# ZPP-Robotics/OSQP-Solver

Hardware: AMD Instinct MI355X
Metric: QPs/sec on a 1024-QP batch of box-QPs (n=512, m=1024), OSQP defaults; ADMM iters/sec alongside (higher is better)
Workload: dtype f64

## Files before the change

### include/mi_osqp.h

```cpp
#ifndef MI_OSQP_H
#define MI_OSQP_H

#include <stdint.h>

#ifdef __cplusplus
extern "C" {
#endif

typedef enum {
  MI_OSQP_OK = 0,
  MI_OSQP_ERR_INVALID_DATA = 1,
  MI_OSQP_ERR_INVALID_SETTINGS = 2,
  MI_OSQP_ERR_PATTERN_CHANGED = 3,
  MI_OSQP_ERR_NONCONVEX = 4,
  MI_OSQP_ERR_DEVICE = 5,
  MI_OSQP_ERR_NULL = 6,
  MI_OSQP_ERR_ALLOC = 7
} mi_osqp_error;

typedef enum {
  MI_OSQP_EXIT_OPTIMAL = 0,
  MI_OSQP_EXIT_PRIMAL_INFEASIBLE = 1,
  MI_OSQP_EXIT_DUAL_INFEASIBLE = 2,
  MI_OSQP_EXIT_OPTIMAL_INACCURATE = 3,
// ... 9 lines not shown
typedef struct {
  double  rho;
  double  sigma;
  int64_t scaling;
  int64_t adaptive_rho;
  int64_t adaptive_rho_interval;
  double  adaptive_rho_tolerance;
  int64_t max_iter;
  double  eps_abs;
  double  eps_rel;
  double  eps_prim_inf;
  double  eps_dual_inf;
  double  alpha;
  int64_t scaled_termination;
  int64_t check_termination;
  int64_t warm_start;
  int64_t verbose;
  int64_t polish;
  int64_t polish_refine_iter;
  double  delta;
} mi_osqp_settings;

typedef struct {
  int64_t iter;
  int64_t status_val;
  int64_t exit_code;
  double  obj_val;
  double  pri_res;
  double  dua_res;
  int64_t rho_updates;
  double  rho_estimate;
  double  rho;
  int64_t status_polish;
} mi_osqp_info;

typedef struct {
  int64_t n, m, N, batch, tile, n_tiles;
  int64_t nnz_P_triu, nnz_A, nnz_KKT, nnz_L;
  int64_t n_supernodes, n_blocks;
  int64_t fwd_levels, bwd_levels, fwd_slots, bwd_slots, chk_slots;
  int64_t lds_bytes, threads_per_block;
  int64_t dense_tail_rows, dense_tail_slots;
  double  setup_seconds_host, setup_seconds_factor, setup_seconds_upload;
  int64_t nnz_L_before_tail;
  int64_t solve_groups, solve_group_threads;
  int64_t resident_state, lds_bytes_iterate;
  int64_t pipelined_refactors;
  int64_t resident_factor_steps, lds_bytes_factor;
  int64_t dense_tail_tasks, dense_tail_waves_used, dense_tail_wave_tasks_max;
  int64_t refactor_lanes;
  int64_t iterate_launches_deep_ring, iterate_launches_long_head;
  int64_t runahead_regions, runahead_tiles, runahead_left, runahead_missed;
  int64_t region_priority, region_lane_checks, region_chunks;
} mi_osqp_stats;

typedef struct mi_osqp_solver mi_osqp_solver;
typedef struct mi_osqp_batch  mi_osqp_batch;

void        mi_osqp_default_settings(mi_osqp_settings *s);
const char *mi_osqp_exit_code_name(int64_t exit_code);
const char *mi_osqp_error_name(int64_t err);
const char *mi_osqp_version(void);
const char *mi_osqp_last_error(void);

int mi_osqp_setup(mi_osqp_solver **out, int64_t n, int64_t m,
                  const int64_t *P_colptr, const int64_t *P_rowidx, const double *P_val,
                  const double *q,
                  const int64_t *A_colptr, const int64_t *A_rowidx, const double *A_val,
                  const double *l, const double *u, const mi_osqp_settings *settings);
int mi_osqp_update_A(mi_osqp_solver *h, const int64_t *A_colptr, const int64_t *A_rowidx,
                     const double *A_val);
int mi_osqp_update_bounds(mi_osqp_solver *h, const double *l, const double *u);
int mi_osqp_update_A_bounds(mi_osqp_solver *h, const int64_t *A_colptr, const int64_t *A_rowidx, const double *A_val,
                            const double *l, const double *u);
int mi_osqp_warm_start_x(mi_osqp_solver *h, const double *x);
int mi_osqp_update_q(mi_osqp_solver *h, const double *q);
int mi_osqp_update_P(mi_osqp_solver *h, const int64_t *P_colptr, const int64_t *P_rowidx, const double *P_val);
int mi_osqp_update_P_A(mi_osqp_solver *h, const int64_t *P_colptr, const int64_t *P_rowidx, const double *P_val,
                       const int64_t *A_colptr, const int64_t *A_rowidx, const double *A_val);
int mi_osqp_warm_start_y(mi_osqp_solver *h, const double *y);
int mi_osqp_solve(mi_osqp_solver *h, mi_osqp_info *info);
int mi_osqp_get_primal(mi_osqp_solver *h, double *x_out);
int mi_osqp_get_dual(mi_osqp_solver *h, double *y_out);
int mi_osqp_get_prim_inf_cert(mi_osqp_solver *h, double *dy_out );
int mi_osqp_get_dual_inf_cert(mi_osqp_solver *h, double *dx_out );
int mi_osqp_adjoint(mi_osqp_solver *h, const double *dx, const double *dy, double *dq, double *dP, double *dA, double *dl, double *du,
                    int32_t *status);
int mi_osqp_get_stats(mi_osqp_solver *h, mi_osqp_stats *st);
int mi_osqp_get_settings(mi_osqp_solver *h, mi_osqp_settings *out);
int mi_osqp_update_settings(mi_osqp_solver *h, const mi_osqp_settings *s);
void mi_osqp_free(mi_osqp_solver *h);

int mi_osqp_batch_setup(mi_osqp_batch **out, int64_t B, int64_t n, int64_t m,
                        const int64_t *P_colptr, const int64_t *P_rowidx, const double *P_val,
                        const double *q,
                        const int64_t *A_colptr, const int64_t *A_rowidx, const double *A_val,
                        const double *l, const double *u, const mi_osqp_settings *settings,
                        int64_t device);
int mi_osqp_batch_update_A(mi_osqp_batch *h, const int64_t *A_colptr, const int64_t *A_rowidx,
                           const double *A_val);
int mi_osqp_batch_update_bounds(mi_osqp_batch *h, const double *l, const double *u);
int mi_osqp_batch_update_A_bounds(mi_osqp_batch *h, const int64_t *A_colptr, const int64_t *A_rowidx, const double *A_val,
                                  const double *l, const double *u);
int mi_osqp_batch_warm_start_x(mi_osqp_batch *h, const double *x);
int mi_osqp_batch_update_q(mi_osqp_batch *h, const double *q);
int mi_osqp_batch_update_P(mi_osqp_batch *h, const int64_t *P_colptr, const int64_t *P_rowidx, const double *P_val);
// ... 117 lines not shown
int mi_osqp_multi_batch_update_rho_each(mi_osqp_multi *h, const double *rho );
int mi_osqp_multi_batch_solve(mi_osqp_multi *h);
int mi_osqp_multi_batch_solve_async(mi_osqp_multi *h);
int mi_osqp_multi_batch_wait(mi_osqp_multi *h);
int mi_osqp_multi_batch_get_primal(mi_osqp_multi *h, double *x_out );
int mi_osqp_multi_batch_get_dual(mi_osqp_multi *h, double *y_out );
int mi_osqp_multi_batch_get_info(mi_osqp_multi *h, mi_osqp_info *info );
int mi_osqp_multi_batch_get_prim_inf_cert(mi_osqp_multi *h, double *dy_out );
int mi_osqp_multi_batch_get_dual_inf_cert(mi_osqp_multi *h, double *dx_out );
int64_t mi_osqp_multi_batch_shards(mi_osqp_multi *h);
int mi_osqp_multi_batch_shard(mi_osqp_multi *h, int64_t k, int64_t *device, int64_t *begin, int64_t *end, mi_osqp_batch **handle);
void mi_osqp_multi_batch_free(mi_osqp_multi *h);

int mi_osqp_batch_spmv(mi_osqp_batch *h, const double *d_x, const double *d_y,
                       double *d_Px, double *d_Aty, double *d_Ax, void *stream);
int mi_osqp_batch_kkt_solve(mi_osqp_batch *h, const double *d_rhs, double *d_sol, void *stream);
int mi_osqp_batch_refactor_device(mi_osqp_batch *h);
int mi_osqp_batch_kernel_time(mi_osqp_batch *h, double *avg_ms, int64_t *launches);
int mi_osqp_batch_refactor_time(mi_osqp_batch *h, double *factor_ms, double *tail_ms, int64_t *launches, int64_t *qps);
int mi_osqp_batch_refactor_peak(mi_osqp_batch *h, int64_t *qps, double *factor_ms, double *tail_ms);

int mi_osqp_batch_get_scaling(mi_osqp_batch *h, double *D , double *E , double *c );

int mi_osqp_debug_host_kkt_solve(int64_t n, int64_t m,
                                 const int64_t *P_colptr, const int64_t *P_rowidx, const double *P_val,
                                 const int64_t *A_colptr, const int64_t *A_rowidx, const double *A_val,
                                 const double *l, const double *u, const mi_osqp_settings *settings,
                                 int64_t tile, const double *rhs ,
                                 double *sol_schedule , double *sol_direct ,
                                 mi_osqp_stats *st);

int mi_osqp_debug_host_block_factor(int64_t n, int64_t m,
                                    const int64_t *P_colptr, const int64_t *P_rowidx, const double *P_val,
                                    const int64_t *A_colptr, const int64_t *A_rowidx, const double *A_val,
                                    const double *l, const double *u, const mi_osqp_settings *settings,
                                    double *max_rel_diff_L, double *max_rel_diff_Dinv, int64_t *counts);

int mi_osqp_debug_refactor_chunks(int64_t n_flagged, const int64_t *flagged, int64_t n_active, const int64_t *active, int64_t tile,
                                  int64_t chunk_qps, int64_t max_chunks, int64_t *n_chunks, int64_t *work_begin, int64_t *tiles,
                                  int64_t *tile_begin);

int mi_osqp_debug_region_chunks(int64_t nq, int64_t gw, int64_t n_cus, int64_t *chunk_qps, int64_t *n_chunks);

int mi_osqp_debug_refactor_lanes(int64_t n_flagged, const int64_t *flagged, int64_t n_active, const int64_t *active, int64_t tile,
                                 int64_t chunk_qps, int64_t max_chunks, int64_t kbt, int64_t lanes, int64_t chunk0_first,
                                 int64_t scratch_slots, int64_t *n_lanes, int64_t *lane_of, int64_t *order, int64_t *order_begin,
                                 int64_t *scratch_begin, int64_t *n_waits, int64_t *wait_chunk, int64_t *wait_for);

int mi_osqp_debug_runahead_group(int64_t n_active, const int64_t *tiles, const double *pri_res, const double *dua_res, int64_t size,
                                 int64_t min_active, int64_t *n_group, int64_t *group);

int mi_osqp_debug_iterate_form(int64_t tiles, int64_t has_head, int64_t forced_form, int64_t long_min, int64_t *form);

int mi_osqp_debug_trace_kkt_solve(mi_osqp_batch *h, int32_t which, const double *d_rhs, double *d_sol,
                                  uint32_t *out, int64_t out_capacity_words, int64_t *dims);

#ifdef __cplusplus
}
#endif
#endif
```

### osqp-solver_amd/__init__.py

```python
import ctypes as C
import os

import numpy as np

try:
    import torch
except ImportError:
    torch = None

from . import build as _build

_HERE = os.path.dirname(os.path.abspath(__file__))
_LIB = None

EXIT_NAMES = ["kOptimal", "kPrimalInfeasible", "kDualInfeasible", "kOptimalInaccurate",
              "kPrimalInfeasibleInaccurate", "kDualInfeasibleInaccurate", "kMaxIterations",
              "kInterrupted", "kTimeLimitReached", "kNonConvex", "kUnknown"]
K_OPTIMAL = 0


class Settings(C.Structure):
    _fields_ = [("rho", C.c_double), ("sigma", C.c_double), ("scaling", C.c_int64),
                ("adaptive_rho", C.c_int64), ("adaptive_rho_interval", C.c_int64),
                ("adaptive_rho_tolerance", C.c_double), ("max_iter", C.c_int64),
                ("eps_abs", C.c_double), ("eps_rel", C.c_double), ("eps_prim_inf", C.c_double),
                ("eps_dual_inf", C.c_double), ("alpha", C.c_double), ("scaled_termination", C.c_int64),
                ("check_termination", C.c_int64), ("warm_start", C.c_int64), ("verbose", C.c_int64),
                ("polish", C.c_int64), ("polish_refine_iter", C.c_int64), ("delta", C.c_double)]


class Info(C.Structure):
    _fields_ = [("iter", C.c_int64), ("status_val", C.c_int64), ("exit_code", C.c_int64),
                ("obj_val", C.c_double), ("pri_res", C.c_double), ("dua_res", C.c_double),
                ("rho_updates", C.c_int64), ("rho_estimate", C.c_double), ("rho", C.c_double),
                ("status_polish", C.c_int64)]

    def as_dict(self):
        return {k: getattr(self, k) for k, _ in self._fields_}


class Stats(C.Structure):
    _fields_ = [(k, C.c_int64) for k in
                ("n", "m", "N", "batch", "tile", "n_tiles", "nnz_P_triu", "nnz_A", "nnz_KKT", "nnz_L",
                 "n_supernodes", "n_blocks", "fwd_levels", "bwd_levels", "fwd_slots", "bwd_slots",
                 "chk_slots", "lds_bytes", "threads_per_block", "dense_tail_rows", "dense_tail_slots")] + \
               [(k, C.c_double) for k in ("setup_seconds_host", "setup_seconds_factor", "setup_seconds_upload")] + \
               [("nnz_L_before_tail", C.c_int64), ("solve_groups", C.c_int64), ("solve_group_threads", C.c_int64),
                ("resident_state", C.c_int64), ("lds_bytes_iterate", C.c_int64), ("pipelined_refactors", C.c_int64),
                ("resident_factor_steps", C.c_int64), ("lds_bytes_factor", C.c_int64),
                ("dense_tail_tasks", C.c_int64), ("dense_tail_waves_used", C.c_int64), ("dense_tail_wave_tasks_max", C.c_int64),
                ("refactor_lanes", C.c_int64),
                ("iterate_launches_deep_ring", C.c_int64), ("iterate_launches_long_head", C.c_int64),
                ("runahead_regions", C.c_int64), ("runahead_tiles", C.c_int64), ("runahead_left", C.c_int64),
                ("runahead_missed", C.c_int64),
                ("region_priority", C.c_int64), ("region_lane_checks", C.c_int64), ("region_chunks", C.c_int64)]

    def as_dict(self):
        return {k: getattr(self, k) for k, _ in self._fields_}


class MiOsqpError(RuntimeError):
    def __init__(self, code, where):
        self.code = int(code)
        L = lib()
        msg = L.mi_osqp_error_name(int(code)).decode()
        extra = L.mi_osqp_last_error().decode()
        super().__init__(f"{where}: error {int(code)} ({msg}) {extra}")


def lib():
    global _LIB
    if _LIB is None:
        path = os.path.join(_HERE, "libmi_osqp.so")
        if os.environ.get("MI_OSQP_LIBRARY"):
            path = os.environ["MI_OSQP_LIBRARY"]
        else:
            try:
                path = _build.build()
            except Exception as e:
                if not os.path.exists(path):
                    raise ImportError(f"libmi_osqp.so missing and could not be built: {e}") from e
        L = C.CDLL(path)
        ip, dp, vp = C.POINTER(C.c_int64), C.POINTER(C.c_double), C.c_void_p
        L.mi_osqp_default_settings.argtypes = [C.POINTER(Settings)]
        for f in ("mi_osqp_exit_code_name", "mi_osqp_error_name"):
            getattr(L, f).restype = C.c_char_p; getattr(L, f).argtypes = [C.c_int64]
        L.mi_osqp_version.restype = C.c_char_p
        L.mi_osqp_last_error.restype = C.c_char_p
        L.mi_osqp_batch_setup.argtypes = [C.POINTER(vp), C.c_int64, C.c_int64, C.c_int64, ip, ip, dp, dp, ip, ip, dp,
                                          dp, dp, C.POINTER(Settings), C.c_int64]
        L.mi_osqp_batch_update_A.argtypes = [vp, ip, ip, dp]
        L.mi_osqp_batch_update_A_bounds.argtypes = [vp, ip, ip, dp, dp, dp]
        L.mi_osqp_batch_update_bounds.argtypes = [vp, dp, dp]
        L.mi_osqp_batch_warm_start_x.argtypes = [vp, dp]
        L.mi_osqp_batch_update_q.argtypes = [vp, dp]
        L.mi_osqp_batch_update_q_device.argtypes = [vp, vp, vp]
        L.mi_osqp_batch_update_P.argtypes = [vp, ip, ip, dp]
        L.mi_osqp_batch_update_P_A.argtypes = [vp, ip, ip, dp, ip, ip, dp]
        L.mi_osqp_batch_warm_start_y.argtypes = [vp, dp]
        L.mi_osqp_batch_get_P_upper_pattern.argtypes = [vp, ip, ip, ip]
        L.mi_osqp_batch_update_P_device.argtypes = [vp, vp, vp]
        L.mi_osqp_batch_update_P_A_bounds_device.argtypes = [vp, vp, vp, vp, vp, vp]
        L.mi_osqp_batch_update_P_some.argtypes = [vp, C.c_int64, ip, dp]
        L.mi_osqp_batch_update_P_A_bounds_some.argtypes = [vp, C.c_int64, ip, dp, dp, dp, dp]
        L.mi_osqp_batch_update_q_some.argtypes = [vp, C.c_int64, ip, dp]
        L.mi_osqp_batch_warm_start_y_some.argtypes = [vp, C.c_int64, ip, dp]
        L.mi_osqp_settings_update_check.argtypes = [C.POINTER(Settings), C.POINTER(Settings)]
        L.mi_osqp_batch_get_settings.argtypes = [vp, C.POINTER(Settings)]
# ... 36 lines not shown
        L.mi_osqp_batch_refactor_peak.argtypes = [vp, ip, dp, dp]
        L.mi_osqp_batch_reinit_some.argtypes = [vp, C.c_int64, ip, dp, dp, dp]
        L.mi_osqp_batch_update_A_bounds_some.argtypes = [vp, C.c_int64, ip, dp, dp, dp]
        L.mi_osqp_batch_warm_start_x_some.argtypes = [vp, C.c_int64, ip, dp]
        L.mi_osqp_batch_solve_begin_some.argtypes = [vp, C.c_int64, ip]
        L.mi_osqp_batch_polish_some.argtypes = [vp, C.c_int64, ip]
        L.mi_osqp_batch_advance.argtypes = [vp, C.c_int64]
        L.mi_osqp_batch_poll.argtypes = [vp, C.c_int64, ip, ip, C.c_int64]
        L.mi_osqp_batch_get_primal_some.argtypes = [vp, C.c_int64, ip, dp]
        L.mi_osqp_batch_get_dual_some.argtypes = [vp, C.c_int64, ip, dp]
        L.mi_osqp_batch_get_info_some.argtypes = [vp, C.c_int64, ip, C.POINTER(Info)]
        L.mi_osqp_batch_running.argtypes = [vp]; L.mi_osqp_batch_running.restype = C.c_int64
        L.mi_osqp_batch_ring_wraps.argtypes = [vp]; L.mi_osqp_batch_ring_wraps.restype = C.c_int64
        L.mi_osqp_release_device_cache.argtypes = []; L.mi_osqp_release_device_cache.restype = None
        L.mi_osqp_setup.argtypes = [C.POINTER(vp), C.c_int64, C.c_int64, ip, ip, dp, dp, ip, ip, dp, dp, dp, C.POINTER(Settings)]
        L.mi_osqp_update_A.argtypes = [vp, ip, ip, dp]
        L.mi_osqp_update_bounds.argtypes = [vp, dp, dp]
        L.mi_osqp_warm_start_x.argtypes = [vp, dp]
        L.mi_osqp_update_q.argtypes = [vp, dp]
        L.mi_osqp_update_P.argtypes = [vp, ip, ip, dp]
        L.mi_osqp_update_P_A.argtypes = [vp, ip, ip, dp, ip, ip, dp]
        L.mi_osqp_warm_start_y.argtypes = [vp, dp]
        L.mi_osqp_solve.argtypes = [vp, C.POINTER(Info)]
        L.mi_osqp_get_primal.argtypes = [vp, dp]
        L.mi_osqp_get_dual.argtypes = [vp, dp]
        L.mi_osqp_get_stats.argtypes = [vp, C.POINTER(Stats)]
        L.mi_osqp_free.argtypes = [vp]; L.mi_osqp_free.restype = None
        L.mi_osqp_multi_batch_setup.argtypes = [C.POINTER(vp), C.c_int64, ip, C.c_int64, C.c_int64, C.c_int64, ip, ip, dp, dp,
                                                ip, ip, dp, dp, dp, C.POINTER(Settings)]
        L.mi_osqp_multi_batch_update_A.argtypes = [vp, ip, ip, dp]
        L.mi_osqp_multi_batch_update_bounds.argtypes = [vp, dp, dp]
        L.mi_osqp_multi_batch_update_A_bounds.argtypes = [vp, ip, ip, dp, dp, dp]
        L.mi_osqp_multi_batch_warm_start_x.argtypes = [vp, dp]
        L.mi_osqp_multi_batch_update_q.argtypes = [vp, dp]
        L.mi_osqp_multi_batch_update_P.argtypes = [vp, ip, ip, dp]
        L.mi_osqp_multi_batch_update_P_A.argtypes = [vp, ip, ip, dp, ip, ip, dp]
        L.mi_osqp_multi_batch_warm_start_y.argtypes = [vp, dp]
        L.mi_osqp_multi_batch_solve.argtypes = [vp]
        L.mi_osqp_multi_batch_solve_async.argtypes = [vp]
        L.mi_osqp_multi_batch_wait.argtypes = [vp]
        L.mi_osqp_multi_batch_get_primal.argtypes = [vp, dp]
        L.mi_osqp_multi_batch_get_dual.argtypes = [vp, dp]
        L.mi_osqp_multi_batch_get_info.argtypes = [vp, C.POINTER(Info)]
        L.mi_osqp_multi_batch_shards.argtypes = [vp]; L.mi_osqp_multi_batch_shards.restype = C.c_int64
        L.mi_osqp_multi_batch_shard.argtypes = [vp, C.c_int64, ip, ip, ip, C.POINTER(vp)]
        L.mi_osqp_multi_batch_free.argtypes = [vp]; L.mi_osqp_multi_batch_free.restype = None
        L.mi_osqp_debug_host_kkt_solve.argtypes = [C.c_int64, C.c_int64, ip, ip, dp, ip, ip, dp, dp, dp,
                                                   C.POINTER(Settings), C.c_int64, dp, dp, dp, C.POINTER(Stats)]
        L.mi_osqp_debug_refactor_chunks.argtypes = [C.c_int64, ip, C.c_int64, ip, C.c_int64, C.c_int64, C.c_int64, ip, ip, ip, ip]
        L.mi_osqp_debug_refactor_lanes.argtypes = [C.c_int64, ip, C.c_int64, ip] + [C.c_int64] * 7 + [ip] * 8
        L.mi_osqp_debug_runahead_group.argtypes = [C.c_int64, ip, dp, dp, C.c_int64, C.c_int64, ip, ip]
        L.mi_osqp_debug_region_chunks.argtypes = [C.c_int64] * 3 + [ip] * 2
        L.mi_osqp_debug_iterate_form.argtypes = [C.c_int64] * 4 + [ip]
        L.mi_osqp_prefetch_analysis.argtypes = [C.c_int64, C.c_int64, C.c_int64, ip, ip, ip, ip, C.c_int64]
        L.mi_osqp_debug_host_block_factor.argtypes = [C.c_int64, C.c_int64, ip, ip, dp, ip, ip, dp, dp, dp,
                                                      C.POINTER(Settings), dp, dp, ip]
        _LIB = L
    return _LIB


def host_cores():
    try:
        n = len(os.sched_getaffinity(0))
    except Exception:
        n = os.cpu_count() or 1
    for path in ("/sys/fs/cgroup/cpu.max",):
        try:
            quota, period = open(path).read().split()[:2]
            if quota != "max":
                n = min(n, max(1, int(round(int(quota) / int(period)))))
        except Exception:
            pass
    try:
        q = int(open("/sys/fs/cgroup/cpu/cpu.cfs_quota_us").read())
        p = int(open("/sys/fs/cgroup/cpu/cpu.cfs_period_us").read())
        if q > 0:
            n = min(n, max(1, int(round(q / p))))
    except Exception:
        pass
    return n


def default_settings(**kw):
    s = Settings()
    lib().mi_osqp_default_settings(C.byref(s))
    for k, v in kw.items():
        if not hasattr(s, k):
            raise KeyError(k)
        setattr(s, k, v)
    return s


class HandleSettings(Settings):

    def bind(self, getter):
        self._getter = getter
        return self

    def __call__(self):
        out = Settings()
        self._getter(out)
        C.memmove(C.byref(self), C.byref(out), C.sizeof(Settings))
        return out


def settings_update_check(in_force, wanted):
# ... 579 lines not shown


def debug_refactor_chunks(flagged, active, tile, chunk_qps, max_chunks=8):
    f, a = _i64(flagged), _i64(active)
    nch = C.c_int64()
    wb = np.zeros(max_chunks + 2, dtype=np.int64); tb = np.zeros(max_chunks + 2, dtype=np.int64)
    tl = np.zeros(max(1, len(a)), dtype=np.int64)
    _chk(lib().mi_osqp_debug_refactor_chunks(len(f), _ip(f), len(a), _ip(a), tile, chunk_qps, max_chunks, C.byref(nch), _ip(wb), _ip(tl),
                                             _ip(tb)), "debug_refactor_chunks")
    k = int(nch.value)
    return ([f[wb[c]:wb[c + 1]].tolist() for c in range(k)], [tl[tb[c]:tb[c + 1]].tolist() for c in range(k)])


def debug_refactor_lanes(flagged, active, tile, chunk_qps, lanes, kbt=None, chunk0_first=False, scratch_slots=None, max_chunks=8):
    f, a = _i64(flagged), _i64(active)
    kbt = tile if kbt is None else kbt
    work, _ = debug_refactor_chunks(flagged, active, tile, chunk_qps, max_chunks)
    k = len(work)
    nl, nw = C.c_int64(), C.c_int64()
    lane_of = np.zeros(max_chunks + 2, dtype=np.int64); order = np.zeros(max_chunks + 2, dtype=np.int64)
    ob = np.zeros(4, dtype=np.int64); sb = np.zeros(max_chunks + 2, dtype=np.int64)
    wc = np.zeros((max_chunks + 1) ** 2, dtype=np.int64); wf = np.zeros((max_chunks + 1) ** 2, dtype=np.int64)
    _chk(lib().mi_osqp_debug_refactor_lanes(len(f), _ip(f), len(a), _ip(a), tile, chunk_qps, max_chunks, kbt, lanes, int(bool(chunk0_first)),
                                            2 ** 31 - 1 if scratch_slots is None else scratch_slots, C.byref(nl), _ip(lane_of), _ip(order),
                                            _ip(ob), _ip(sb), C.byref(nw), _ip(wc), _ip(wf)), "debug_refactor_lanes")
    L = int(nl.value)
    return dict(n_lanes=L, lane_of=lane_of[:k].tolist(), order=[order[ob[l]:ob[l + 1]].tolist() for l in range(L)],
                scratch=[(int(sb[c]), (len(work[c]) + kbt - 1) // kbt * kbt) for c in range(k)],
                waits=list(zip(wc[:nw.value].tolist(), wf[:nw.value].tolist())))


def debug_region_chunks(nq, gw, n_cus):
    q, k = C.c_int64(), C.c_int64()
    _chk(lib().mi_osqp_debug_region_chunks(nq, gw, n_cus, C.byref(q), C.byref(k)), "debug_region_chunks")
    return int(q.value), int(k.value)


def debug_runahead_group(tiles, pri_res, dua_res, size, min_active):
    t, p, d = _i64(tiles), _f64(pri_res), _f64(dua_res)
    if not (len(t) == len(p) == len(d)):
        raise ValueError("tiles, pri_res and dua_res differ in length")
    ng = C.c_int64()
    out = np.zeros(max(1, len(t)), dtype=np.int64)
    _chk(lib().mi_osqp_debug_runahead_group(len(t), _ip(t), _dp(p), _dp(d), size, min_active, C.byref(ng), _ip(out)), "debug_runahead_group")
    return out[:ng.value].tolist()


def debug_iterate_form(tiles, has_head=True, forced_form=0, long_min=-1):
    form = C.c_int64()
    _chk(lib().mi_osqp_debug_iterate_form(tiles, int(bool(has_head)), forced_form, long_min, C.byref(form)), "debug_iterate_form")
    return int(form.value)


def debug_host_block_factor(P, A, l, u, **settings):
    L = lib()
    P, A = _csc(P), _csc(A)
    n, m = A.shape[1], A.shape[0]
    s = default_settings(**settings)
    Pp, Pi, Px = _i64(P.indptr), _i64(P.indices), _f64(P.data)
    Ap, Ai, Ax = _i64(A.indptr), _i64(A.indices), _f64(A.data)
    l, u = _f64(l), _f64(u)
    dL, dD = C.c_double(), C.c_double()
    cnt = (C.c_int64 * 4)()
    rc = L.mi_osqp_debug_host_block_factor(n, m, _ip(Pp), _ip(Pi), _dp(Px), _ip(Ap), _ip(Ai), _dp(Ax), _dp(l), _dp(u),
                                           C.byref(s), C.byref(dL), C.byref(dD), cnt)
    _chk(rc, "debug_host_block_factor")
    return dL.value, dD.value, dict(blocks=cnt[0], triples=cnt[1], storage=cnt[2], levels=cnt[3])
```

### osqp-solver_amd/csrc/device_types.h

```cpp
#pragma once
#include <hip/hip_runtime.h>
#include <stdint.h>

namespace miosqp {

#define MI_CHUNK 16

struct SchedDev {
  const uint32_t *step, *idxw;
  const uint64_t *idxw64;
  const uint32_t *lvl_pos, *tail_bar;
  int n_phases, nw, n_levels;
  uint32_t n_steps, n_slots;
};

struct DenseTailDev {
  int s, k, n_phases;
  uint32_t n_steps;
  const uint32_t *task;
  const uint32_t *wave_task, *wave_step, *tail_bar;
};

enum { DS_C = 0, DS_CINV, DS_RHO, DS_RHO_EST, DS_PRI_RES, DS_DUA_RES, DS_OBJ, DS_COUNT };
enum { IS_STATUS = 0, IS_ITER, IS_RHO_UPDATES, IS_DONE, IS_NEED_REFACTOR, IS_CUR, IS_PENDING, IS_EPOCH, IS_COUNT };

enum { RF_FORM_NONE = 0, RF_FORM_DEEP_RING = 1, RF_FORM_LONG_HEAD = 2 };

struct KernelArgs {
  int n, m, N, B;
  SchedDev fwd, bwd, chk;
  const uint32_t *pinv;
  const uint32_t *xloc;
  const double *fwd_val, *bwd_val, *chk_val, *dinv;
  DenseTailDev dt;
  const double *dt_val;
  const double *fwd_val0, *bwd_val0, *dt_val0;
  const int *use_work;
  double *x, *z, *y;
  const double *q, *l, *u, *rho_vec, *rho_inv, *Dsc, *Dsc_inv, *Esc, *Esc_inv;
  double *dx, *dy, *out1, *out2, *dscal;
  int *iscal;
  double *x_out, *y_out;
  double *cert_out;
  int cert_stride;
  double *xs_global;
  int xs_len;
  int rs_off;
  int rf_off;
  int rf_form;
  int wide;
  double sigma, alpha, eps_abs, eps_rel, eps_prim_inf, eps_dual_inf, rho_tolerance;
  int check_termination, rho_interval, max_iter, scaled_termination, scaling, adaptive_rho;
  int iter_begin, iter_end;
  int op_out_lds;
  int info_at_end;
  int mw_groups;
  unsigned *mw_bar;
  double *mw_scratch;
  int df;
  unsigned df_shadow;
  const unsigned char *rflag;
  const int *sel;
  const int *tiles;
  double *res;
};

struct FactorArgs {
  int n, m, N, B, nnzP, nnzK, pa_len, n_levels, force_all;
  int debug_skip;
  uint32_t storage;
  SchedDev fwd, bwd;
  const uint32_t *blk, *lvl, *utask, *tri4, *dtask, *ttask, *asm_dst, *asm_src;
  const uint32_t *ubig;
  int *use_work;
  const int32_t *fwd_srcblk, *bwd_srcblk;
  const double *pa_val, *l, *u, *dscal;
  double *rho_vec, *rho_inv, *Lblk, *Dl, *dinv_scratch, *fwd_val, *bwd_val, *dinv;
  int *iscal, *npos;
  int home_bt;
  const int *work;
  int wg_base;
  double sigma;
  int dt_k;
  int mw_groups;
  unsigned *mw_bar;
  const signed char *pmask;
  const int32_t *arow;
  int *pstat;
  double pdelta;
};

struct TailArgs {
  int n, N, s, k, kbt, home_bt;
  uint32_t storage, n_slots;
  int n_lt, n_ltcol;
  uint32_t n_quads;
  int nh;
  uint32_t cs_doubles;
  const int *work;
  int wg_base;
  const uint32_t *lt_pos, *ltcol_col, *tile_tab, *wave_tiles, *diag_tile;
  const uint64_t *asm_q64;
// ... 126 lines not shown
```

### osqp-solver_amd/csrc/host_core.cpp

```cpp
#include "host_core.hpp"
#include "sched_format.h"

#include <algorithm>
#include <cmath>
#include <cstdio>
#include <cstdlib>
#include <cstring>
#include <limits>
#include <numeric>
#include <set>
#include <chrono>
#include <thread>

#include "../../include/mi_osqp.h"

namespace miosqp {

int validate_settings(const Settings &s) {
  if (s.scaling < 0 || s.max_iter <= 0 || s.check_termination < 0) return 1;
  if (s.adaptive_rho != 0 && s.adaptive_rho != 1) return 1;
  if (s.adaptive_rho_interval < 0 || s.adaptive_rho_tolerance < 1.0) return 1;
  if (!(s.rho > 0.0) || !(s.sigma > 0.0)) return 1;
  if (s.eps_abs < 0.0 || s.eps_rel < 0.0 || (s.eps_abs == 0.0 && s.eps_rel == 0.0)) return 1;
  if (!(s.eps_prim_inf > 0.0) || !(s.eps_dual_inf > 0.0)) return 1;
// ... 882 lines not shown
        }
        const uint32_t blk_id = find_blk(ct0 + t.I, ct0 + t.J);
        dt.tile_tab.insert(dt.tile_tab.end(), {((uint32_t)t.I << 16) | (uint32_t)t.J, bf.blk[4 * blk_id], q0, (uint32_t)(dt.asm_q.size() / 64)});
      }
    }
    dt.wave_tiles[nw] = (uint32_t)(dt.tile_tab.size() / 4);
    dt.asm_q64.resize(dt.asm_q.size());
    for (size_t e = 0; e < dt.asm_q.size(); e++) {
      const uint64_t w = dt.asm_q[e], ci = dt.asm_qcol[e / 16];
      dt.asm_q64[e] = ((w & 0xFFFFu) * 8u) | ((((w >> 16) * 8u) | ((ci * 8u) << 17)) << 32);
    }
    dt.src_tile.resize(dt.src.size());
    for (size_t e = 0; e < dt.src.size(); e++) {
      const int32_t sc = dt.src[e];
      dt.src_tile[e] = sc < 0 ? sc : (int32_t)dt_tile_offset(sc % k, sc / k);
    }
    dt.diag_tile.resize(k);
    for (int i = 0; i < k; i++) dt.diag_tile[i] = dt_tile_offset(i, i);
    dt.task_step.clear();
    { uint32_t pos = 0; for (size_t t = 0; t < dt.task.size() / 4; t++) { dt.task_step.push_back(pos); pos += dt.task[4 * t + 3]; } }
  }
}


Tuning tuning_from_env() {
  Tuning t;
  if (const char *e = getenv("MI_OSQP_TILE")) { const int v = atoi(e); if (v == 1 || v == 2 || v == 4) t.tile = v; }
  if (const char *e = getenv("MI_OSQP_THREADS")) t.threads = std::max(64, std::min(1024, atoi(e) / 64 * 64));
  t.global_xs = getenv("MI_OSQP_GLOBAL_XS") != nullptr;
  if (const char *e = getenv("MI_OSQP_GROUPS")) t.groups = std::max(0, std::min(256, atoi(e)));
  if (const char *e = getenv("MI_OSQP_GROUP_THREADS")) t.group_threads = std::max(64, std::min(512, atoi(e) / 64 * 64));
  if (const char *e = getenv("MI_OSQP_ASSUME_CUS")) t.assume_cus = std::max(0, atoi(e));
  if (const char *e = getenv("MI_OSQP_FACTOR_THREADS")) t.factor_threads = std::max(64, std::min(1024, atoi(e) / 64 * 64));
  if (const char *e = getenv("MI_OSQP_FACTOR_GROUPS")) t.factor_groups = std::max(1, std::min(256, atoi(e)));
  t.ruiz = getenv("MI_OSQP_HOST_RUIZ") ? 1 : getenv("MI_OSQP_DEVICE_RUIZ") ? -1 : 0;
  if (const char *e = getenv("MI_OSQP_CONT_RING_KB")) t.cont_ring_kb = std::max(0L, atol(e));
  if (const char *e = getenv("MI_OSQP_ANALYSIS_CACHE")) t.analysis_cache = atoi(e) != 0;
  t.stream_state = getenv("MI_OSQP_STREAM_STATE") != nullptr;
  t.stream_factor = getenv("MI_OSQP_STREAM_FACTOR") != nullptr;
  if (const char *e = getenv("MI_OSQP_REFACTOR_PIPELINE")) t.refactor_pipeline = atoi(e) != 0;
  if (const char *e = getenv("MI_OSQP_REFACTOR_PIPELINE_MIN")) t.pipeline_min = std::max(0, atoi(e));
  if (const char *e = getenv("MI_OSQP_REFACTOR_CHUNKS")) t.pipeline_chunks = std::max(0, std::min(8, atoi(e)));
  if (const char *e = getenv("MI_OSQP_REFACTOR_CHUNK_QPS")) t.pipeline_chunk_qps = std::max(0, atoi(e));
  if (const char *e = getenv("MI_OSQP_REFACTOR_LANES")) t.refactor_lanes = std::max(1, std::min(3, atoi(e)));
  if (const char *e = getenv("MI_OSQP_REFACTOR_CHUNK0")) t.lanes_chunk0 = atoi(e) != 0;
  if (const char *e = getenv("MI_OSQP_REGION_PRIORITY")) t.region_priority = std::max(0, std::min(2, atoi(e)));
  if (const char *e = getenv("MI_OSQP_LANE_CHECKS")) t.lane_checks = atoi(e) != 0;
  if (const char *e = getenv("MI_OSQP_RUNAHEAD")) t.runahead = atoi(e) != 0;
  if (const char *e = getenv("MI_OSQP_RUNAHEAD_TILES")) t.runahead_tiles = std::max(0, atoi(e));
  if (const char *e = getenv("MI_OSQP_RUNAHEAD_MIN")) t.runahead_min = std::max(0, atoi(e));
  if (const char *e = getenv("MI_OSQP_RUNAHEAD_END")) t.runahead_end = std::max(0, atoi(e));
  if (const char *e = getenv("MI_OSQP_RF_FORM")) { const int v = atoi(e); if (v == kIterDeepRing || v == kIterLongHead) t.rf_form = v; }
  if (const char *e = getenv("MI_OSQP_RF_LONG_MIN")) t.rf_long_min = std::max(0, atoi(e));
  AnalysisTuning &a = t.analysis;
  if (const char *e = getenv("MI_OSQP_DENSE_TAIL")) a.dense_tail = atoi(e);
  if (const char *e = getenv("MI_OSQP_ORDERING")) a.ordering = e[0];
  if (const char *e = getenv("MI_OSQP_ND_LEAF")) a.nd_leaf = atoi(e);
  if (const char *e = getenv("MI_OSQP_RELAX")) a.relax = atoi(e);
  a.serial = getenv("MI_OSQP_SERIAL_ANALYSIS") != nullptr;
  return t;
}

RefactorChunks refactor_chunks(const std::vector<int> &flagged, const std::vector<int> &active, int bt, int chunk_qps, int max_chunks) {
  RefactorChunks rc;
  const int nq = (int)flagged.size();
  max_chunks = std::max(1, max_chunks);
  chunk_qps = std::max(1, chunk_qps);
  if ((nq + chunk_qps - 1) / chunk_qps > max_chunks) chunk_qps = (nq + max_chunks - 1) / max_chunks;
  const int n_ref = (nq + chunk_qps - 1) / chunk_qps;
  rc.n_chunks = 1 + n_ref;
  rc.work_begin.assign(1, 0);
  for (int c = 0; c <= n_ref; c++) rc.work_begin.push_back(std::min(nq, c * chunk_qps));
  std::vector<std::pair<int, int>> tc;
  size_t f = 0;
  for (size_t i = 0; i < active.size(); i++) {
    const int tile = active[i] / bt;
    if (i && active[i - 1] / bt == tile) continue;
    int chunk = 0;
    while (f < flagged.size() && flagged[f] / bt < tile) f++;
    for (size_t g = f; g < flagged.size() && flagged[g] / bt == tile; g++) chunk = 1 + (int)g / chunk_qps;
    tc.emplace_back(chunk, tile);
  }
  std::stable_sort(tc.begin(), tc.end(), [](const std::pair<int, int> &x, const std::pair<int, int> &y) { return x.first < y.first; });
  rc.tile_begin.assign((size_t)rc.n_chunks + 1, 0);
  for (const auto &p : tc) { rc.tiles.push_back(p.second); rc.tile_begin[(size_t)p.first + 1]++; }
  for (int c = 0; c < rc.n_chunks; c++) rc.tile_begin[(size_t)c + 1] += rc.tile_begin[c];
  return rc;
}

int region_chunk_qps(int nq, int gw, int n_cus, int max_chunks) {
  nq = std::max(0, nq); gw = std::max(0, gw); n_cus = std::max(1, n_cus);
  const int64_t rounds = ((int64_t)nq + gw + n_cus - 1) / n_cus;
  const int64_t want = gw > 0 ? 2 * rounds - 1 : rounds;
  const int n_even = (int)std::max<int64_t>(1, std::min<int64_t>(want, std::min(std::max(1, max_chunks), std::max(1, nq))));
  return (int)std::max<int64_t>(1, ((int64_t)nq + n_even - 1) / n_even);
}

RefactorLanes refactor_lanes(const RefactorChunks &ch, const std::vector<int> &flagged, int bt, int kbt, int lanes, bool chunk0_first, int scratch_slots) {
  RefactorLanes rl;
  const int nc = ch.n_chunks, n_ref = nc - 1;
  bt = std::max(1, bt); kbt = std::max(1, kbt);
  int L = std::max(1, std::min(std::min(3, lanes), std::max(1, n_ref)));
  std::vector<int> padded((size_t)nc + 1, 0);
  for (int c = 1; c < nc; c++) padded[(size_t)c + 1] = padded[c] + (ch.work_begin[(size_t)c + 1] - ch.work_begin[c] + kbt - 1) / kbt * kbt;
  if (padded[nc] > scratch_slots) L = 1;
  rl.n_lanes = L;
// ... 6 lines not shown
  }
  rl.scratch_begin = padded;
  for (int c = 1; c < nc; c++) { rl.lane_of[c] = (c - 1) % L; rl.order[(c - 1) % L].push_back(c); }
  if (chunk0_first) { rl.lane_of[0] = L - 1; rl.order[L - 1].insert(rl.order[L - 1].begin(), 0); }
  else {
    int at = L - 1;
    for (int a = L - 1; a >= 0; a--) if (rl.order[a].size() < rl.order[at].size()) at = a;
    rl.lane_of[0] = at; rl.order[at].push_back(0);
  }
  for (int c = 1; c < nc; c++) {
    std::vector<char> need(nc, 0);
    for (int t = ch.tile_begin[c]; t < ch.tile_begin[(size_t)c + 1]; t++) {
      const int tile = ch.tiles[t];
      size_t g = std::lower_bound(flagged.begin(), flagged.end(), tile * bt) - flagged.begin();
      for (; g < flagged.size() && flagged[g] / bt == tile; g++) {
        const int d = (int)(std::upper_bound(ch.work_begin.begin() + 1, ch.work_begin.end(), (int)g) - ch.work_begin.begin()) - 1;
        if (d >= 1 && d < c && rl.lane_of[d] != rl.lane_of[c]) need[d] = 1;
      }
    }
    for (int d = 1; d < c; d++) if (need[d]) { rl.wait_chunk.push_back(c); rl.wait_for.push_back(d); }
  }
  return rl;
}

std::vector<int> runahead_group(const std::vector<int> &tiles, const std::vector<double> &pri, const std::vector<double> &dua, int size, int min_active) {
  const size_t na = tiles.size();
  if (!na || size <= 0 || na < (size_t)std::max(0, min_active) || pri.size() != na || dua.size() != na) return {};
  const double inf = std::numeric_limits<double>::infinity();
  auto scaled = [&](const std::vector<double> &r) {
    std::vector<double> v(na);
    for (size_t i = 0; i < na; i++) v[i] = std::isnan(r[i]) ? inf : r[i];
    std::vector<double> s = v;
    std::nth_element(s.begin(), s.begin() + na / 2, s.end());
    const double med = s[na / 2];
    for (size_t i = 0; i < na; i++) v[i] = v[i] == inf ? inf : med == inf ? 0.0 : med > 0.0 ? v[i] / med : v[i] > 0.0 ? inf : 0.0;
    return v;
  };
  const std::vector<double> sp = scaled(pri), sd = scaled(dua);
  std::vector<std::pair<double, int>> order(na);
  for (size_t i = 0; i < na; i++) order[i] = {sp[i] + sd[i], tiles[i]};
  std::sort(order.begin(), order.end(), [](const std::pair<double, int> &x, const std::pair<double, int> &y) {
    return x.first > y.first || (x.first == y.first && x.second < y.second);
  });
  std::vector<int> group(std::min(na, (size_t)size));
  for (size_t i = 0; i < group.size(); i++) group[i] = order[i].second;
  return group;
}

int iterate_form(int tiles, bool has_head, const Tuning &t) {
  if (!has_head) return kIterStreamed;
  if (t.rf_form == kIterDeepRing || t.rf_form == kIterLongHead) return t.rf_form;
  const int long_min = t.rf_long_min >= 0 ? t.rf_long_min : kRfLongMinDefault;
  return tiles > 0 && tiles >= long_min ? kIterLongHead : kIterDeepRing;
}


int analyze(int64_t n64, int64_t m64, const int64_t *Pp, const int64_t *Pi, const int64_t *Ap,
            const int64_t *Ai, const AnalysisTuning &tune, Analysis &an, int nwaves, int bt, int max_extra_rows, int dense_tail_max, int tri_waves, int n_tiles) {
  if (nwaves < 1 || nwaves > 16 || (bt != 1 && bt != 2 && bt != 4) || tri_waves < 0 || tri_waves > 2048) return MI_OSQP_ERR_INVALID_SETTINGS;
  if (n64 <= 0 || m64 < 0 || !Pp || !Ap || n64 + m64 > (int64_t)1 << 30) return MI_OSQP_ERR_INVALID_DATA;
  int n = (int)n64, m = (int)m64, N = n + m;
  an = Analysis();
  an.n = n; an.m = m; an.N = N;
  if (Pp[0] != 0 || Ap[0] != 0) return MI_OSQP_ERR_INVALID_DATA;
  for (int j = 0; j < n; j++) {
    if (Pp[j + 1] < Pp[j] || Ap[j + 1] < Ap[j]) return MI_OSQP_ERR_INVALID_DATA;
    for (int64_t k = Pp[j]; k < Pp[j + 1]; k++) if (Pi[k] < 0 || Pi[k] >= n) return MI_OSQP_ERR_INVALID_DATA;
    for (int64_t k = Ap[j]; k < Ap[j + 1]; k++) if (Ai[k] < 0 || Ai[k] >= m) return MI_OSQP_ERR_INVALID_DATA;
  }
  if (Pp[n] > (int64_t)1 << 30 || Ap[n] > (int64_t)1 << 30) return MI_OSQP_ERR_INVALID_DATA;
  an.Pp.assign(n + 1, 0);
  for (int j = 0; j < n; j++) {
    an.Pp[j] = (int)an.Pi.size();
    for (int64_t k = Pp[j]; k < Pp[j + 1]; k++)
      if (Pi[k] <= j) { an.Pi.push_back((int)Pi[k]); an.Psrc.push_back((int)k); }
  }
  an.Pp[n] = (int)an.Pi.size();
  an.Ap.assign(Ap, Ap + n + 1);
  an.Ai.assign(Ai, Ai + Ap[n]);
  int nnzP = an.Pp[n], nnzA = an.Ap[n];
  std::vector<int> cnt(N, 0);
  an.PisDiag.assign(nnzP, 0);
  std::vector<char> hasDiag(n, 0);
  for (int j = 0; j < n; j++)
    for (int k = an.Pp[j]; k < an.Pp[j + 1]; k++) { cnt[j]++; if (an.Pi[k] == j) { hasDiag[j] = 1; an.PisDiag[k] = 1; } }
  for (int j = 0; j < n; j++) if (!hasDiag[j]) cnt[j]++;
  for (int k = 0; k < nnzA; k++) cnt[n + an.Ai[k]]++;
  for (int r = 0; r < m; r++) cnt[n + r]++;
  an.Kp.assign(N + 1, 0);
  for (int j = 0; j < N; j++) an.Kp[j + 1] = an.Kp[j] + cnt[j];
  an.Ki.assign(an.Kp[N], 0);
  an.PtoK.assign(nnzP, 0); an.AtoK.assign(nnzA, 0); an.rhotoK.assign(m, 0);
  std::vector<int> nxt(an.Kp.begin(), an.Kp.end() - 1);
  for (int j = 0; j < n; j++) {
    for (int k = an.Pp[j]; k < an.Pp[j + 1]; k++) { int pos = nxt[j]++; an.Ki[pos] = an.Pi[k]; an.PtoK[k] = pos; }
    if (!hasDiag[j]) { int pos = nxt[j]++; an.Ki[pos] = j; an.sigmaOnlyK.push_back(pos); }
  }
  for (int j = 0; j < n; j++)
    for (int k = an.Ap[j]; k < an.Ap[j + 1]; k++) { int pos = nxt[n + an.Ai[k]]++; an.Ki[pos] = j; an.AtoK[k] = pos; }
  for (int r = 0; r < m; r++) { int pos = nxt[n + r]++; an.Ki[pos] = n + r; an.rhotoK[r] = pos; }
  an.tri_waves = tri_waves;
  an.wide = N >= 65535 || 2 * n + m >= 65535 || tri_waves > 0;
  if (max_extra_rows < 0) max_extra_rows = 1 << 30;
  if (!an.wide && max_extra_rows > 65534 - N) max_extra_rows = 65534 - N;
  auto finalize = [&](Analysis &an, const std::vector<int> &perm0, double &cost, int relax_zeros = 0, int *phases_out = nullptr, double *stream_out = nullptr) {
    an.perm = perm0;
// ... 742 lines not shown
```

### osqp-solver_amd/csrc/host_core.hpp

```cpp
#pragma once

#include <cstdint>
#include <string>
#include <vector>

namespace miosqp {

constexpr double kInfty = 1e30;
constexpr double kRhoMin = 1e-6, kRhoMax = 1e6, kRhoEqOverIneq = 1e3, kRhoTol = 1e-4;
constexpr double kMinScaling = 1e-4, kMaxScaling = 1e4;
constexpr double kDivisionTol = 1.0 / kInfty;
constexpr int kChunk = 16;
constexpr uint32_t kNoRow = 0xFFFFFFFFu;

struct Settings {
  double rho = 0.1, sigma = 1e-6;
  int64_t scaling = 10, adaptive_rho = 1, adaptive_rho_interval = 0;
  double adaptive_rho_tolerance = 5.0;
  int64_t max_iter = 4000;
  double eps_abs = 1e-3, eps_rel = 1e-3, eps_prim_inf = 1e-4, eps_dual_inf = 1e-4, alpha = 1.6;
  int64_t scaled_termination = 0, check_termination = 25, warm_start = 1, verbose = 0;
  int64_t polish = 0, polish_refine_iter = 3;
  double delta = 1e-6;
};
int validate_settings(const Settings &s);

struct AnalysisTuning {
  int dense_tail = -1;
  char ordering = 0;
  int nd_leaf = 0;
  int relax = -1;
  bool serial = false;
  bool operator==(const AnalysisTuning &o) const {
    return dense_tail == o.dense_tail && ordering == o.ordering && nd_leaf == o.nd_leaf && relax == o.relax && serial == o.serial;
  }
};
constexpr bool kRunaheadDefault = true;
constexpr int kRegionPriorityDefault = 0;
constexpr bool kLaneChecksDefault = false;
struct Tuning {
  int tile = 0;
  int threads = 0;
  bool global_xs = false;
  int groups = -1;
  int group_threads = 0;
  int assume_cus = 0;
  int factor_threads = 1024;
  int factor_groups = 0;
  int ruiz = 0;
  long cont_ring_kb = -1;
  bool analysis_cache = true;
  bool stream_state = false;
  bool stream_factor = false;
  bool refactor_pipeline = true;
  int pipeline_min = 0;
  int pipeline_chunks = 0;
  int pipeline_chunk_qps = 0;
  int refactor_lanes = 0;
  int lanes_chunk0 = -1;
  int region_priority = kRegionPriorityDefault;
  bool lane_checks = kLaneChecksDefault;
  bool runahead = kRunaheadDefault;
  int runahead_tiles = 0;
  int runahead_min = 0;
  int runahead_end = 0;
  int rf_form = 0;
  int rf_long_min = -1;
  AnalysisTuning analysis;
};
Tuning tuning_from_env();

enum IterateForm { kIterStreamed = 0, kIterDeepRing = 1, kIterLongHead = 2 };
constexpr int kRfLongMinDefault = 0;
int iterate_form(int tiles, bool has_head, const Tuning &t);

struct RefactorChunks {
  int n_chunks = 1;
  std::vector<int> work_begin;
  std::vector<int> tiles;
  std::vector<int> tile_begin;
};
RefactorChunks refactor_chunks(const std::vector<int> &flagged, const std::vector<int> &active, int bt, int chunk_qps, int max_chunks);

int region_chunk_qps(int nq, int gw, int n_cus, int max_chunks);

struct RefactorLanes {
  int n_lanes = 1;
  std::vector<int> lane_of;
  std::vector<std::vector<int>> order;
  std::vector<int> scratch_begin;
  std::vector<int> wait_chunk, wait_for;
};
RefactorLanes refactor_lanes(const RefactorChunks &ch, const std::vector<int> &flagged, int bt, int kbt, int lanes, bool chunk0_first, int scratch_slots);

std::vector<int> runahead_group(const std::vector<int> &tiles, const std::vector<double> &pri, const std::vector<double> &dua, int size, int min_active);

struct Schedule {
  int n_phases = 0, nw = 0, bt = 1;
  bool barriers = true;
  std::vector<uint32_t> phase;
  std::vector<int> level_first_phase;
  std::vector<uint32_t> step;
  std::vector<uint32_t> step_ob;
  std::vector<uint32_t> outA;
  std::vector<uint32_t> idx;
  std::vector<uint32_t> idxw;
  std::vector<uint64_t> idxw64;
  std::vector<int32_t> src;
  uint32_t n_slots = 0;
  uint32_t n_steps = 0;
  std::vector<uint32_t> wave_range;
  std::vector<uint32_t> lvl_pos;
  std::vector<uint32_t> tail_bar;
  bool dataflow = false;
  uint32_t shadow = 0, pad = 0;
  uint32_t phys_steps() const { return n_steps; }
  size_t phase_stride() const { return 4 * (size_t)nw + 1; }
  int n_levels = 0;
};

struct BlockFactor {
  uint32_t storage = 0;
  std::vector<uint32_t> blk;
// ... 120 lines not shown
```

### osqp-solver_amd/csrc/kernels.hip

```cpp
#include <hip/hip_runtime.h>
#include <stdint.h>
#include <stdlib.h>
#include <string.h>

#include <algorithm>
#include <map>
#include <mutex>

#include "device_types.h"
#include "sched_format.h"

namespace miosqp {

static hipError_t ensure_dynamic_lds(const void *kern, size_t lds);

#define MI_INFTY 1e30
#define MI_MIN_SCALING 1e-4
#define MI_DIV_TOL 1e-30
#define MI_RHO_EST_DIV 1e-10
#define MI_RHO_MIN 1e-6
#define MI_RHO_MAX 1e6
#define MI_NOROW 0xFFFFFFFFu
#ifdef MI_OSQP_DEBUG_BUILD
#define MI_DBG_SKIP(a) ((a).debug_skip)
// ... 127 lines not shown
    const bool o0 = lane & 1;
    const double sd = o0 ? acc[0] : acc[1];
    kp = o0 ? acc[1] : acc[0];
    kp += dpp_d<DPP_XOR1>(sd);
    if (lt > 1) kp += dpp_d<DPP_SHL(2)>(kp);
    if (lt > 2) kp += dpp_d<DPP_SHL(4)>(kp);
    if (lt > 3) kp += dpp_d<DPP_SHL(8)>(kp);
  } else {
    kp = acc[0];
    kp += dpp_d<DPP_SHL(1)>(kp);
    if (lt > 1) kp += dpp_d<DPP_SHL(2)>(kp);
    if (lt > 2) kp += dpp_d<DPP_SHL(4)>(kp);
    if (lt > 3) kp += dpp_d<DPP_SHL(8)>(kp);
  }
  if (lt > 4) kp += down16_d(kp);
  if (lt > 5) kp += down32_d(kp);
  if (has_row && ((uint32_t)lane & (T - 1)) < (uint32_t)BT)
    base[(size_t)row * BT + flush_q<BT>(lane)] = sub ? oldv[0] - kp : kp;
}

#ifndef MI_PFV
#define MI_PFV 9
#endif
#define MI_PFV_OF(BT, GX) MI_PFV
#ifndef MI_PFV_LAT
#define MI_PFV_LAT 6
#endif
#define MI_PFV_NT(NT, GX) (((NT) > 512 && !(GX)) ? MI_PFV_LAT : MI_PFV)
template <int BT, int PF>
struct Ring { double v[PF][BT]; uint32_t gi[PF]; uint32_t gr[PF]; uint32_t desc; };
template <int BT>
struct ValSrc { mi_rsrc vals[BT], idx, step; };

template <int BT, bool WIDE>
__device__ __forceinline__ void load_step(const ValSrc<BT> &vs, uint32_t stepno, int lane, double (&v)[BT], uint32_t &gi, uint32_t &gr) {
  if constexpr (WIDE) {
    const mi_u32x2 t = __builtin_amdgcn_raw_buffer_load_b64(vs.idx, (uint32_t)lane * 8u, stepno * 512u, 0);
    gi = t.x; gr = t.y;
  } else {
    gi = __builtin_amdgcn_raw_buffer_load_b32(vs.idx, (uint32_t)lane * 4u, stepno * 256u, 0);
  }
#pragma unroll
  for (int b = 0; b < BT; b++) {
    const mi_u32x2 t = __builtin_amdgcn_raw_buffer_load_b64(vs.vals[b], (uint32_t)lane * 8u, stepno * 512u, 0);
    v[b] = __hiloint2double((int)t.y, (int)t.x);
  }
}
template <int BT>
__device__ __forceinline__ uint32_t load_desc(const ValSrc<BT> &vs, uint32_t pos, uint32_t end, int lane) {
  const uint32_t d = __builtin_amdgcn_raw_buffer_load_b32(vs.step, (uint32_t)lane * 4u, pos * 4u, 0);
  return pos + (uint32_t)lane < end ? d : MI_D_NOOP;
}

template <int BT, int PF, bool SUB, bool BAR, bool GX, int TR = 0, bool WIDE = false>
__device__ __forceinline__ void run_stream(const ValSrc<BT> &vs, uint32_t begin, uint32_t end, uint32_t tail, double *xs,
                                           double *out, int lane, uint32_t *tr = nullptr, int wave = 0, int nw = 0,
                                           uint32_t *tw = nullptr) {
  double *base = SUB ? xs : out;
  Ring<BT, PF> r;
  r.desc = MI_D_NOOP;
#pragma unroll
  for (int st = 0; st < PF; st++) {
    r.gi[st] = 0u; r.gr[st] = 0u;
#pragma unroll
    for (int b = 0; b < BT; b++) r.v[st][b] = 0.0;
  }
  constexpr uint32_t NONE = WIDE ? 0xFFFFFFFFu : 0xFFFFu;
  static_assert(PF % (MI_D_LOOKAHEAD + 1) == 0, "the gather slots must line up across ring revolutions");
  constexpr int GS = MI_D_LOOKAHEAD + 1;
  double acc[BT], xq[GS][BT];
#pragma unroll
  for (int b = 0; b < BT; b++) {
    acc[b] = 0.0;
#pragma unroll
    for (int g = 0; g < GS; g++) xq[g][b] = 0.0;
  }
  uint32_t nbar_seen = 0, wait_cycles = 0, real_steps = 0;
  auto barrier = [&]() {
    if constexpr (TR) { if (lane == 0) tr[((size_t)nbar_seen * nw + wave) * 2] = (uint32_t)__builtin_amdgcn_s_memtime(); }
    if constexpr (GX) __syncthreads(); else lds_barrier();
    if constexpr (TR) { if (lane == 0) tr[((size_t)nbar_seen * nw + wave) * 2 + 1] = (uint32_t)__builtin_amdgcn_s_memtime(); nbar_seen++; }
  };
  for (uint32_t npos = begin; npos < end + PF; npos += PF) {
    const uint32_t dnext = load_desc(vs, npos, end, lane);
#pragma unroll
    for (int st = 0; st < PF; st++) {
      const uint32_t d = (uint32_t)__builtin_amdgcn_readlane((int)r.desc, st);
      if constexpr (BAR) { for (uint32_t nb = MI_D_NBAR(d); nb; nb--) barrier(); }
      const uint32_t type = MI_D_TYPE(d);
      if constexpr (TR >= 2) {
        if (type != 3u) {
          const uint32_t t0 = (uint32_t)__builtin_amdgcn_s_memtime();
          asm volatile("s_waitcnt vmcnt(29)" ::: "memory");
          wait_cycles += (uint32_t)__builtin_amdgcn_s_memtime() - t0;
          real_steps++;
        }
      }
      if (type == MI_D_TYPE_ROW) {
        const uint32_t w = r.gi[st];
        if (!(d & MI_D_PRE)) load_bt<BT>(xs + (size_t)(WIDE ? w : (w & 0xFFFFu)) * BT, xq[st % GS]);
        const bool sub = SUB && !(d & MI_D_STORE);
        const bool flush = d & MI_D_FLUSH;
        double oldv[BT];
        const uint32_t lt = MI_D_LT(d), row = WIDE ? r.gr[st] : (w >> 16);
        if (flush && sub) flush_prefetch<BT, NONE>(lt, row, base, lane, oldv);
        if (d & MI_D_AHEAD) {
          const int s2 = (st + MI_D_LOOKAHEAD) % PF;
          load_bt<BT>(xs + (size_t)(WIDE ? r.gi[s2] : (r.gi[s2] & 0xFFFFu)) * BT, xq[(st + MI_D_LOOKAHEAD) % GS]);
        }
#pragma unroll
        for (int b = 0; b < BT; b++) acc[b] = fma(r.v[st][b], xq[st % GS][b], acc[b]);
        if (flush) {
          reduce_write<BT, NONE>(acc, lt, row, base, lane, sub, oldv);
#pragma unroll
          for (int b = 0; b < BT; b++) acc[b] = 0.0;
        }
      }
      load_step<BT, WIDE>(vs, npos + (uint32_t)st, lane, r.v[st], r.gi[st], r.gr[st]);
    }
    r.desc = dnext;
  }
  if constexpr (BAR) { for (uint32_t nb = tail; nb; nb--) barrier(); }
  if constexpr (TR >= 2) { if (lane == 0) { tw[2 * wave] = wait_cycles; tw[2 * wave + 1] = real_steps; } }
}

#define MI_GX_PF 18
#define MI_GX_LA 8
struct Mw { unsigned *bar; unsigned G; };
__device__ __forceinline__ void grid_barrier(const Mw &mw) {
  __syncthreads();
  if (threadIdx.x == 0 && !__hip_atomic_load(&mw.bar[2], __ATOMIC_RELAXED, __HIP_MEMORY_SCOPE_AGENT)) {
    __builtin_amdgcn_fence(__ATOMIC_RELEASE, "agent");
    asm volatile("s_waitcnt vmcnt(0)" ::: "memory");
    const unsigned gen = __hip_atomic_load(&mw.bar[1], __ATOMIC_RELAXED, __HIP_MEMORY_SCOPE_AGENT);
    const unsigned arrived = __hip_atomic_fetch_add(&mw.bar[0], 1u, __ATOMIC_RELAXED, __HIP_MEMORY_SCOPE_AGENT) + 1u;
    if (arrived == mw.G) {
// ... 108 lines not shown
      oq[sj % G] = ld_sc1(xs + (mine ? row : 0u));
    };
#pragma unroll
    for (int st = 0; st < PF; st++) {
      const uint32_t d = (uint32_t)__builtin_amdgcn_readlane((int)r.desc, st);
      const uint32_t dl = st + LA < PF ? (uint32_t)__builtin_amdgcn_readlane((int)r.desc, (st + LA) % PF)
                                       : (uint32_t)__builtin_amdgcn_readlane((int)dnext, (st + LA) % PF);
      request(st + LA, dl);
      if (MI_D_TYPE(d) == MI_D_TYPE_ROW) {
        double xv = xq[st % G];
        if (__builtin_amdgcn_ballot_w64(__double_as_longlong(xv) == MI_DF_NOTYET) && !dead) {
          const unsigned long long t0 = __builtin_amdgcn_s_memrealtime();
          uint32_t spins = 0;
          do {
            xv = ld_sc1(xs + r.gi[st]);
            if ((++spins & 63u) == 0u &&
                (__builtin_amdgcn_s_memrealtime() - t0 > 200000000ull || __hip_atomic_load(err, __ATOMIC_RELAXED, __HIP_MEMORY_SCOPE_AGENT))) {
              __hip_atomic_store(err, 1u, __ATOMIC_RELAXED, __HIP_MEMORY_SCOPE_AGENT);
              dead = true;
              break;
            }
          } while (__builtin_amdgcn_ballot_w64(__double_as_longlong(xv) == MI_DF_NOTYET));
        }
        acc = fma(r.v[st][0], xv, acc);
        if (d & MI_D_FLUSH) {
          const uint32_t lt = MI_D_LT(d), row = r.gr[st];
          const bool sub = !(d & MI_D_STORE);
          double kp = acc;
          if (lt > 0) kp += dpp_d<DPP_SHL(1)>(kp);
          if (lt > 1) kp += dpp_d<DPP_SHL(2)>(kp);
          if (lt > 2) kp += dpp_d<DPP_SHL(4)>(kp);
          if (lt > 3) kp += dpp_d<DPP_SHL(8)>(kp);
          if (lt > 4) kp += down16_d(kp);
          if (lt > 5) kp += down32_d(kp);
          if (row != 0xFFFFFFFFu && ((uint32_t)lane & ((1u << lt) - 1u)) == 0u)
            st_sc1(xs + (size_t)row + (sub ? shadow : 0u), sub ? oq[st % G] - kp : kp);
          acc = 0.0;
        }
      }
      load_step<1, true>(vs, npos + (uint32_t)st, lane, r.v[st], r.gi[st], r.gr[st]);
    }
    r.desc = dnext;
  }
}

template <int BT, int PF, bool GX, int TR = 0, bool WIDE = false>
__device__ __forceinline__ void run_tri(const SchedDev &s, const ValSrc<BT> &vals, double *xs, int wave, int lane,
                                        uint32_t *tr = nullptr, uint32_t *tw = nullptr) {
  mi_cptr lp = as_const(s.lvl_pos);
  const uint32_t begin = lp[wave], end = lp[(size_t)s.n_levels * s.nw + wave], tail = as_const(s.tail_bar)[wave];
  if constexpr (GX && TR == 0 && BT <= 2) run_stream_gx<BT, MI_GX_PF, MI_GX_LA, WIDE>(vals, begin, end, tail, xs, lane);
  else run_stream<BT, PF, true, true, GX, TR, WIDE>(vals, begin, end, tail, xs, nullptr, lane, tr, wave, s.nw, tw);
}

template <int BT, int PF, bool WIDE = false>
__device__ __forceinline__ void run_spmv(const SchedDev &s, const ValSrc<BT> &vals, double *xs, double *out, int wave,
                                         int lane, int l0, int l1, int nwaves_here = 0) {
  mi_cptr lp = as_const(s.lvl_pos);
  const int step = nwaves_here > 0 ? nwaves_here : (int)s.nw;
  for (int vw = wave; vw < (int)s.nw; vw += step) {
    const uint32_t begin = lp[(size_t)l0 * s.nw + vw], end = lp[(size_t)l1 * s.nw + vw];
    run_stream<BT, PF, false, false, false, 0, WIDE>(vals, begin, end, 0u, xs, out, lane);
  }
}

template <int BT, int K, bool IS_MAX>
__device__ __forceinline__ void block_reduce(double (&v)[K], double *red, int tid, int wave, int nw, int lane) {
#pragma unroll
  for (int k = 0; k < K; k++) {
#pragma unroll
    for (int off = BT; off < 64; off <<= 1) {
      const double o = shfl_xor_d(v[k], off);
      v[k] = IS_MAX ? fmax(v[k], o) : v[k] + o;
    }
  }
  if (lane < BT) {
#pragma unroll
    for (int k = 0; k < K; k++) red[(wave * K + k) * BT + lane] = v[k];
  }
  __syncthreads();
  double *res = red + nw * K * BT;
  if (tid < K * BT) {
    const int k = tid / BT, b = tid % BT;
    double r = red[k * BT + b];
    for (int w = 1; w < nw; w++) {
      const double o = red[(w * K + k) * BT + b];
      r = IS_MAX ? fmax(r, o) : r + o;
    }
    res[k * BT + b] = r;
  }
  __syncthreads();
#pragma unroll
  for (int k = 0; k < K; k++) v[k] = res[k * BT + (tid % BT)];
  __syncthreads();
}

template <int K, bool IS_MAX>
__device__ __forceinline__ void grid_reduce(double (&v)[K], double *red, const Mw &mw, double *scratch, int ltid, int lwave, int lnw, int lane) {
  if (mw.G <= 1) return;
  if (ltid == 0) {
#pragma unroll
    for (int k = 0; k < K; k++) __hip_atomic_store(scratch + (size_t)blockIdx.x * 16 + k, v[k], __ATOMIC_RELAXED, __HIP_MEMORY_SCOPE_AGENT);
  }
  grid_barrier(mw);
  double w[K];
#pragma unroll
// ... 104 lines not shown
#pragma unroll
      for (int b = 0; b < NQ; b++) { accr[b] = 0.0; accc[b] = 0.0; }
    }
#pragma unroll
    for (int st = 0; st < PF; st++) {
#pragma unroll
      for (int b = 0; b < NQ; b++) {
        accc[b] = fma(rv[st][b], ti[b], accc[b]);
        accr[b] = fma(rv[st][b], tj[b], accr[b]);
      }
#pragma unroll
      for (int b = 0; b < NQ; b++) { ti[b] = rol1_d(ti[b]); accr[b] = rol1_d(accr[b]); }
#pragma unroll
      for (int b = 0; b < NQ; b++) {
        const mi_u32x2 w = __builtin_amdgcn_raw_buffer_load_b64(vals[b], (uint32_t)lane * 8u, (pos + (uint32_t)st) * 512u, 0);
        rv[st][b] = __hiloint2double((int)w.y, (int)w.x);
      }
    }
    if (pos > begin) {
      left -= PF;
      if (left == 0) {
        const uint32_t il = ((uint32_t)lane + (flags & 1u) + nst) & 63u;
        double *rvec = (flags & 2u) ? yc : yr, *cvec = (flags & 2u) ? yr : yc;
#pragma unroll
        for (int b = 0; b < NQ; b++) {
          const int bb = NQ == BT ? b : b0;
          rvec[(size_t)(I0 + il) * BT + bb] += accr[b];
          cvec[(size_t)(J0 + (uint32_t)lane) * BT + bb] += accc[b];
        }
        t++;
      }
    }
  }
  for (uint32_t nb = as_const(dt.tail_bar)[wave]; nb; nb--) lds_barrier();
}

#ifndef MI_RF_RL
#define MI_RF_RL 8
#endif
#ifndef MI_RF_R_DEEP
#define MI_RF_R_DEEP 8
#endif
#ifndef MI_RF_PF_DEEP
#define MI_RF_PF_DEEP (2 * MI_DT_PF)
#endif
#ifndef MI_RF_R_LONG
#define MI_RF_R_LONG 24
#endif
#ifndef MI_RF_PF_LONG
#define MI_RF_PF_LONG 8
#endif
__host__ __device__ constexpr int rf_reg_steps(int RF) { return RF == RF_FORM_LONG_HEAD ? MI_RF_R_LONG : RF == RF_FORM_DEEP_RING ? MI_RF_R_DEEP : 1; }
__host__ __device__ constexpr int rf_ring_steps(int RF) { return RF == RF_FORM_LONG_HEAD ? MI_RF_PF_LONG : MI_RF_PF_DEEP; }
template <int R, int RL, int PF>
__device__ __forceinline__ void dense_tail_apply_rf(const DenseTailDev &dt, const mi_rsrc &vals, const double *xt, double *yr, double *yc,
                                                    double (&keep)[R], double *hl, bool first, int wave, int lane) {
  constexpr int H = R + RL;
  static_assert(H % PF == 0 && H <= 32 && RL <= PF, "the head is whole ring revolutions inside the shortest task");
  mi_cptr tk = as_const(dt.task);
  uint32_t t = as_const(dt.wave_task)[wave];
  const uint32_t begin = as_const(dt.wave_step)[wave], end = as_const(dt.wave_step)[wave + 1];
  if (begin < end) {
    double rv[PF], tj, ti, accr = 0.0, accc = 0.0;
    uint32_t I0 = tk[4 * t], J0 = tk[4 * t + 1], nst = tk[4 * t + 3], flags;
    auto ld = [&](uint32_t step) {
      const mi_u32x2 w = __builtin_amdgcn_raw_buffer_load_b64(vals, (uint32_t)lane * 8u, step * 512u, 0);
      return __hiloint2double((int)w.y, (int)w.x);
    };
    auto fma_step = [&](double v) {
      accc = fma(v, ti, accc);
      accr = fma(v, tj, accr);
      ti = rol1_d(ti); accr = rol1_d(accr);
    };
    auto flush = [&]() {
      const uint32_t il = ((uint32_t)lane + (flags & 1u) + nst) & 63u;
      double *rvec = (flags & 2u) ? yc : yr, *cvec = (flags & 2u) ? yr : yc;
      rvec[I0 + il] += accr;
      cvec[J0 + (uint32_t)lane] += accc;
      t++;
    };
    {
      const uint32_t fl = tk[4 * t + 2];
      for (uint32_t nb = fl >> 8; nb; nb--) lds_barrier();
      flags = fl & 255u;
      tj = xt[J0 + (uint32_t)lane];
      ti = xt[I0 + (((uint32_t)lane + (flags & 1u)) & 63u)];
    }
    if (first) {
#pragma unroll
      for (int st = 0; st < RL; st++) rv[st] = ld(begin + (uint32_t)st);
#pragma unroll
      for (int st = 0; st < R; st++) keep[st] = ld(begin + (uint32_t)(RL + st));
#pragma unroll
      for (int st = 0; st < RL; st++) hl[st * 64] = rv[st];
    } else {
#pragma unroll
      for (int st = 0; st < RL; st++) rv[st] = hl[st * 64];
    }
#pragma unroll
    for (int st = 0; st < RL; st++) fma_step(rv[st]);
    const uint32_t p0 = begin + (uint32_t)H;
    if (p0 < end) {
#pragma unroll
      for (int st = 0; st < PF; st++) rv[st] = ld(p0 + (uint32_t)st);
    }
#pragma unroll
    for (int st = 0; st < R; st++) fma_step(keep[st]);
    uint32_t left = nst - (uint32_t)H;
    if (left == 0) flush();
    for (uint32_t pos = p0 + PF; pos < end + PF; pos += PF) {
      if (left == 0) {
        I0 = tk[4 * t]; J0 = tk[4 * t + 1]; nst = tk[4 * t + 3];
        const uint32_t fl = tk[4 * t + 2];
        for (uint32_t nb = fl >> 8; nb; nb--) lds_barrier();
        flags = fl & 255u; left = nst;
        tj = xt[J0 + (uint32_t)lane];
        ti = xt[I0 + (((uint32_t)lane + (flags & 1u)) & 63u)];
        accr = 0.0; accc = 0.0;
      }
      if (pos < end) {
#pragma unroll
        for (int st = 0; st < PF; st++) { fma_step(rv[st]); rv[st] = ld(pos + (uint32_t)st); }
      } else {
#pragma unroll
        for (int st = 0; st < PF; st++) fma_step(rv[st]);
      }
      left -= PF;
      if (left == 0) flush();
    }
  }
  for (uint32_t nb = as_const(dt.tail_bar)[wave]; nb; nb--) lds_barrier();
}

template <int BT, bool GX>
__device__ __forceinline__ void kkt_middle(const KernelArgs &a, const double *dinv, const mi_rsrc (&vdt)[BT], int act, double *xs,
                                           int tid, int nthr, int wave, int lane) {
  if (!a.dt.k) {
    constexpr int U = GX ? 8 : 1;
    const int tot = a.N * BT;
    for (int e0 = tid; e0 < tot; e0 += nthr * U) {
      size_t pos[U]; double v[U], dv[U];
#pragma unroll
      for (int u = 0; u < U; u++) { const int e = e0 + u * nthr < tot ? e0 + u * nthr : e0; pos[u] = (size_t)a.xloc[e / BT] * BT + e % BT; dv[u] = dinv[e]; }
#pragma unroll
      for (int u = 0; u < U; u++) v[u] = xs[pos[u]];
#pragma unroll
      for (int u = 0; u < U; u++) if (e0 + u * nthr < tot) xs[pos[u]] = v[u] * dv[u];
    }
    __syncthreads();
    return;
  }
  if constexpr (!GX) {
    const int s = a.dt.s, k = a.dt.k;
    double *yr = xs + (size_t)a.xs_len * BT, *yc = yr + (size_t)k * BT;
    for (int e = tid; e < a.N * BT; e += nthr) {
      const int i = e / BT;
      if (i < s) xs[(size_t)a.xloc[i] * BT + e % BT] *= dinv[e];
      else { yr[e - s * BT] = dinv[e] * xs[e]; yc[e - s * BT] = 0.0; }
    }
    __syncthreads();
    if constexpr (BT == 1) {
      dense_tail_apply<1, 1, 2 * MI_DT_PF>(a.dt, vdt, 0, xs + (size_t)s * BT, yr, yc, wave, lane);
    } else {
      const int act_u = __builtin_amdgcn_readfirstlane(act);
      if (BT == 2 && (act_u == 1 || act_u == 2)) {
        const mi_rsrc one[1] = {act_u == 2 ? vdt[BT - 1] : vdt[0]};
        dense_tail_apply<BT, 1, 2 * MI_DT_PF>(a.dt, one, act_u == 2 ? 1 : 0, xs + (size_t)s * BT, yr, yc, wave, lane);
      } else {
        dense_tail_apply<BT, BT, MI_DT_PF>(a.dt, vdt, 0, xs + (size_t)s * BT, yr, yc, wave, lane);
      }
    }
    for (int e = tid; e < k * BT; e += nthr) xs[(size_t)s * BT + e] = yr[e] + yc[e];
    __syncthreads();
  }
}

template <int R, int RL, int PF>
__device__ __forceinline__ void kkt_middle_rf(const KernelArgs &a, const double *dinv, const mi_rsrc &vdt, double *xs, double (&keep)[R],
                                              double *hl, bool first, int tid, int nthr, int wave, int lane) {
  const int s = a.dt.s, k = a.dt.k;
  double *yr = xs + (size_t)a.xs_len, *yc = yr + (size_t)k;
  int e0 = tid;
  asm volatile("" : "+v"(e0));
  for (int e = e0; e < a.N; e += nthr) {
    if (e < s) xs[(size_t)a.xloc[e]] *= dinv[e];
    else { yr[e - s] = dinv[e] * xs[e]; yc[e - s] = 0.0; }
  }
  __syncthreads();
  dense_tail_apply_rf<R, RL, PF>(a.dt, vdt, xs + (size_t)s, yr, yc, keep, hl, first, wave, lane);
  for (int e = tid; e < k; e += nthr) xs[(size_t)s + e] = yr[e] + yc[e];
  __syncthreads();
}

__device__ __forceinline__ uint32_t df_floc(uint32_t e, uint32_t f, uint32_t xl, uint32_t sh) { return (f & 4u) ? xl : ((f & 1u) ? e + sh : e); }
__device__ __forceinline__ uint32_t df_bloc(uint32_t e, uint32_t f, uint32_t sh) { return (f & 4u) ? e : ((f & 2u) ? e + sh : e); }
__device__ __forceinline__ void df_arm_fwd(double *xs, uint32_t e, uint32_t f, uint32_t xl, uint32_t sh) {
  if (f & 1u) st_sc1(xs + e + sh, df_notyet());
  if (f & 4u) st_sc1(xs + xl, df_notyet());
}

template <int BT, int PF, bool GX, bool WIDE = false>
__device__ __forceinline__ void kkt_solve_lds(const KernelArgs &a, const TilePtrs<BT> &p, double *xs,
                                              int tid, int nthr, int wave, int nw, int lane, const Mw &mw = Mw{nullptr, 1u}) {
  if constexpr (GX && BT == 1 && WIDE) {
    if (a.df) {
      mi_cptr lpf = as_const(a.fwd.lvl_pos), lpb = as_const(a.bwd.lvl_pos);
      run_stream_df<MI_GX_PF, MI_GX_LA>(p.vfwd, lpf[wave], lpf[(size_t)a.fwd.n_levels * a.fwd.nw + wave], xs, a.df_shadow, lane, mw.bar + 2);
      wg_or_grid_barrier(mw);
      const uint32_t sh = a.df_shadow;
      constexpr int U = 8;
      for (int e0 = tid; e0 < a.N; e0 += nthr * U) {
        uint32_t xl[U], f[U]; double v[U], dv[U];
#pragma unroll
        for (int u = 0; u < U; u++) { const int e = e0 + u * nthr < a.N ? e0 + u * nthr : e0; xl[u] = a.xloc[e]; f[u] = a.rflag[e]; dv[u] = p.dinv[e]; }
#pragma unroll
        for (int u = 0; u < U; u++) { const int e = e0 + u * nthr < a.N ? e0 + u * nthr : e0; v[u] = ld_sc1(xs + df_floc((uint32_t)e, f[u], xl[u], sh)); }
#pragma unroll
        for (int u = 0; u < U; u++) {
          const int e = e0 + u * nthr;
          if (e < a.N) {
            st_sc1(xs + xl[u], v[u] * dv[u]);
            if (f[u] & 2u) st_sc1(xs + xl[u] + sh, df_notyet());
            if (f[u] & 4u) st_sc1(xs + e, df_notyet());
          }
        }
      }
      wg_or_grid_barrier(mw);
      run_stream_df<MI_GX_PF, MI_GX_LA>(p.vbwd, lpb[wave], lpb[(size_t)a.bwd.n_levels * a.bwd.nw + wave], xs, a.df_shadow, lane, mw.bar + 2);
      wg_or_grid_barrier(mw);
      return;
    }
  }
  run_tri<BT, PF, GX, 0, WIDE>(a.fwd, p.vfwd, xs, wave, lane);
  kkt_middle<BT, GX>(a, p.dinv, p.vdt, p.act, xs, tid, nthr, wave, lane);
  run_tri<BT, PF, GX, 0, WIDE>(a.bwd, p.vbwd, xs, wave, lane);
}

template <int BT, int NT, bool GX, bool WIDE = false, bool RS = false, int RF = 0>
__device__ __forceinline__ void iterate_body(const KernelArgs &a, double *smem, int n_iter) {
  static_assert(!RS || (!GX && !WIDE), "the resident state goes with the LDS solve vector");
  static_assert(!RF || (RS && BT == 1 && NT == 1024), "the resident head goes with the resident state of a 16-wave tile of one QP");
  const Mw mw{a.mw_bar, GX && BT == 1 && a.mw_groups > 1 ? (unsigned)a.mw_groups : 1u};
  const bool multi = GX && BT == 1 && mw.G > 1;
  const int tile = multi ? 0 : (a.tiles ? a.tiles[blockIdx.x] : (int)blockIdx.x);
  const int tid = multi ? blockIdx.x * blockDim.x + threadIdx.x : threadIdx.x, nthr = multi ? blockDim.x * mw.G : blockDim.x;
  const int lane = tid & 63, wave = __builtin_amdgcn_readfirstlane(tid >> 6), nw = nthr >> 6;
  const int b = tid % BT;
  const int n = a.n, m = a.m, N = a.N;
  double *unused_scratch;
  double *xs = solve_vector<BT, GX>(a, smem, tile, unused_scratch);
  const TilePtrs<BT> p = tile_ptrs<BT>(a, tile, true);
  const int done = p.iscal[IS_DONE * BT + b] | (p.iscal[IS_NEED_REFACTOR * BT + b] < 0);
  if (__syncthreads_and(done)) return;
  const double alpha = a.alpha, sigma = a.sigma;
  bool df = false;
  if constexpr (GX && BT == 1 && WIDE) df = a.df != 0;
  const uint32_t sh = a.df_shadow;
  double *rs = nullptr;
  if constexpr (RS) rs = smem + a.rs_off;
  double *const X = RS ? rs : p.x, *const Z = RS ? rs + (size_t)2 * n * BT : p.z, *const Y = RS ? Z + (size_t)m * BT : p.y;
  const double *const Q = RS ? X + (size_t)n * BT : p.q, *const RI = RS ? Y + (size_t)m * BT : p.rho_inv;
  const double *const RV = RS ? RI + (size_t)m * BT : p.rho_vec, *const LO = RS ? RV + (size_t)m * BT : p.l;
  const double *const UP = RS ? LO + (size_t)m * BT : p.u, *const DI = RS ? UP + (size_t)m * BT : p.dinv;
  double keep[rf_reg_steps(RF)];
#pragma unroll
  for (int st = 0; st < rf_reg_steps(RF); st++) keep[st] = 0.0;
  double *hl = nullptr;
  (void)keep; (void)hl;
  if constexpr (RF) hl = smem + a.rf_off + (size_t)(wave * MI_RF_RL) * 64 + lane;
  for (int e = tid; e < N * BT; e += nthr) {
    const int i = e / BT;
    double v;
    if constexpr (RS) {
      rs[(size_t)(2 * n + 6 * m) * BT + e] = p.dinv[e];
      if (i < n) { const double xv = p.x[e], qv = p.q[e]; rs[e] = xv; rs[(size_t)n * BT + e] = qv; v = sigma * xv - qv; }
      else {
        const int ez = e - n * BT;
        const double zv = p.z[ez], ri = p.rho_inv[ez], yv = p.y[ez];
        double *sz = rs + (size_t)2 * n * BT + ez;
        sz[0] = zv; sz[(size_t)m * BT] = yv; sz[(size_t)2 * m * BT] = ri;
        sz[(size_t)3 * m * BT] = p.rho_vec[ez]; sz[(size_t)4 * m * BT] = p.l[ez]; sz[(size_t)5 * m * BT] = p.u[ez];
        v = zv - ri * yv;
      }
    } else {
      if (i < n) v = sigma * p.x[e] - p.q[e];
      else { const int ez = e - n * BT; v = p.z[ez] - p.rho_inv[ez] * p.y[ez]; }
    }
    const uint32_t pe = a.pinv[i];
    if (df) { st_sc1(xs + pe, v); df_arm_fwd(xs, pe, a.rflag[pe], a.xloc[pe], sh); }
    else xs[(size_t)pe * BT + b] = v;
  }
  if (df && tid == 0) st_sc1(xs + 2 * (size_t)sh, 0.0);
  if constexpr (GX) wg_or_grid_barrier(mw); else __syncthreads();
  for (int iter = 1; iter <= n_iter; iter++) {
    const bool do_info = a.info_at_end && iter == n_iter;
    const bool last = iter == n_iter;
    if constexpr (RS) {
      run_tri<BT, MI_PFV_NT(NT, GX), GX, 0, WIDE>(a.fwd, p.vfwd, xs, wave, lane);
      if constexpr (RF) kkt_middle_rf<rf_reg_steps(RF), MI_RF_RL, rf_ring_steps(RF)>(a, DI, p.vdt[0], xs, keep, hl, iter == 1, tid, nthr, wave, lane);
      else kkt_middle<BT, GX>(a, DI, p.vdt, p.act, xs, tid, nthr, wave, lane);
      run_tri<BT, MI_PFV_NT(NT, GX), GX, 0, WIDE>(a.bwd, p.vbwd, xs, wave, lane);
    } else {
      kkt_solve_lds<BT, MI_PFV_NT(NT, GX), GX, WIDE>(a, p, xs, tid, nthr, wave, nw, lane, mw);
    }
    constexpr int U = GX ? 4 : 1;
    int tid_i = tid;
    if constexpr (RF != 0) asm volatile("" : "+v"(tid_i));
    uint32_t fl[U], xl[U];
    for (int e0 = tid_i; e0 < n * BT; e0 += nthr * U) {
      size_t pos[U]; double xt[U], xp[U], qv[U];
#pragma unroll
      for (int u = 0; u < U; u++) { const int e = e0 + u * nthr < n * BT ? e0 + u * nthr : e0; pos[u] = (size_t)a.pinv[e / BT] * BT + b; }
      if (df) {
#pragma unroll
        for (int u = 0; u < U; u++) { fl[u] = a.rflag[pos[u]]; xl[u] = a.xloc[pos[u]]; }
      }
#pragma unroll
      for (int u = 0; u < U; u++) {
        const int e = e0 + u * nthr < n * BT ? e0 + u * nthr : e0;
        xt[u] = df ? ld_sc1(xs + df_bloc((uint32_t)pos[u], fl[u], sh)) : xs[pos[u]]; xp[u] = X[e]; qv[u] = Q[e];
      }
#pragma unroll
      for (int u = 0; u < U; u++) {
        const int e = e0 + u * nthr;
        if (e < n * BT) {
          double xn = alpha * xt[u] + (1.0 - alpha) * xp[u];
          if (!done) {
            X[e] = xn;
            if constexpr (RS) { if (last) p.x[e] = xn; }
            if (do_info) p.dx[e] = xn - xp[u];
          } else xn = xp[u];
          if (df) { st_sc1(xs + pos[u], sigma * xn - qv[u]); df_arm_fwd(xs, (uint32_t)pos[u], fl[u], xl[u], sh); }
          else xs[pos[u]] = sigma * xn - qv[u];
        }
      }
    }
    for (int e0 = tid_i; e0 < m * BT; e0 += nthr * U) {
      size_t pos[U]; double nu[U], zp[U], yv[U], ri[U], rv[U], lo[U], up[U];
#pragma unroll
      for (int u = 0; u < U; u++) { const int e = e0 + u * nthr < m * BT ? e0 + u * nthr : e0; pos[u] = (size_t)a.pinv[n + e / BT] * BT + b; }
      if (df) {
#pragma unroll
        for (int u = 0; u < U; u++) { fl[u] = a.rflag[pos[u]]; xl[u] = a.xloc[pos[u]]; }
      }
#pragma unroll
      for (int u = 0; u < U; u++) {
        const int e = e0 + u * nthr < m * BT ? e0 + u * nthr : e0;
        nu[u] = df ? ld_sc1(xs + df_bloc((uint32_t)pos[u], fl[u], sh)) : xs[pos[u]]; zp[u] = Z[e]; yv[u] = Y[e]; ri[u] = RI[e]; rv[u] = RV[e]; lo[u] = LO[e]; up[u] = UP[e];
      }
#pragma unroll
      for (int u = 0; u < U; u++) {
        const int e = e0 + u * nthr;
        if (e < m * BT) {
          double zt = zp[u] - ri[u] * yv[u];
          zt += ri[u] * nu[u];
          const double zr = alpha * zt + (1.0 - alpha) * zp[u];
          double zn = fmin(fmax(zr + ri[u] * yv[u], lo[u]), up[u]);
          const double dyv = rv[u] * (zr - zn);
          double yn = yv[u] + dyv;
          if (!done) {
            Z[e] = zn; Y[e] = yn;
            if constexpr (RS) { if (last) { p.z[e] = zn; p.y[e] = yn; } }
            if (do_info) p.dy[e] = dyv;
          } else { zn = zp[u]; yn = yv[u]; }
          if (df) { st_sc1(xs + pos[u], zn - ri[u] * yn); df_arm_fwd(xs, (uint32_t)pos[u], fl[u], xl[u], sh); }
          else xs[pos[u]] = zn - ri[u] * yn;
        }
      }
    }
    if constexpr (GX) wg_or_grid_barrier(mw); else __syncthreads();
  }
}
template <int BT, int NT, bool GX, bool WIDE = false, bool RS = false, int RF = 0>
__global__ __launch_bounds__(NT) void iterate_kernel(KernelArgs a) {
  extern __shared__ double smem[];
  iterate_body<BT, NT, GX, WIDE, RS, RF>(a, smem, a.iter_end - a.iter_begin);
}

template <int BT, int NT, bool GX, bool WIDE = false>
__device__ __forceinline__ int check_body(const KernelArgs &a, double *smem, int n_iter) {
  bool dfm = false;
  if constexpr (GX && BT == 1 && WIDE) dfm = a.df != 0 && a.mw_groups > 1;
  const Mw mw{a.mw_bar, dfm ? (unsigned)a.mw_groups : 1u};
  const int tile = dfm ? 0 : (a.tiles ? a.tiles[blockIdx.x] : (int)blockIdx.x);
  const int ltid = threadIdx.x, lwave = __builtin_amdgcn_readfirstlane(ltid >> 6), lnw = blockDim.x >> 6;
  const int tid = dfm ? blockIdx.x * blockDim.x + threadIdx.x : threadIdx.x, nthr = dfm ? blockDim.x * mw.G : blockDim.x;
  const int lane = tid & 63, wave = __builtin_amdgcn_readfirstlane(tid >> 6), nw = nthr >> 6;
  const int b = tid % BT;
  auto sync = [&]() { if constexpr (GX && BT == 1 && WIDE) wg_or_grid_barrier(mw); else __syncthreads(); };
  auto gscratch = [&](int slot) { return a.mw_scratch + (size_t)slot * 256 * 16; };
  const int n = a.n, m = a.m;
  double *red;
  double *xs = solve_vector<BT, GX>(a, smem, tile, red);
  const TilePtrs<BT> p = tile_ptrs<BT>(a, tile, true);
  int done = p.iscal[IS_DONE * BT + b];
  if (__syncthreads_and(done)) return 0;
  const int iter = p.iscal[IS_CUR * BT + b] + n_iter;
  int status = p.iscal[IS_STATUS * BT + b];
  int rho_updates = p.iscal[IS_RHO_UPDATES * BT + b];
  double rho = p.dscal[DS_RHO * BT + b];
  const double c = p.dscal[DS_C * BT + b], cinv = p.dscal[DS_CINV * BT + b];
  const bool unscale = a.scaling && !a.scaled_termination;
  const bool is_last = iter >= a.max_iter;
  const bool is_check = a.check_termination && (iter % a.check_termination == 0);
  const bool is_rho = a.adaptive_rho && a.rho_interval && (iter % a.rho_interval == 0);
  bool any_check = is_check || is_last, any_last = is_last;
  if constexpr (BT > 1) { any_check = __syncthreads_or(any_check); any_last = __syncthreads_or(any_last); }
  int need_refactor = 0;
  for (int e = tid; e < n * BT; e += nthr) xs[e] = p.x[e];
  for (int e = tid; e < m * BT; e += nthr) xs[(size_t)n * BT + e] = p.y[e];
  sync();
  run_spmv<BT, MI_PFV, WIDE>(a.chk, p.vchk, xs, p.out1, wave, lane, 0, 3, nw);
  sync();
  double mx[14];
#pragma unroll
  for (int k = 0; k < 14; k++) mx[k] = 0.0;
  double sm[1] = {0.0};
  for (int e = tid; e < n * BT; e += nthr) {
    const double px = p.out1[e], aty = p.out1[(size_t)n * BT + e], qv = p.q[e], xv = p.x[e];
    const double di = p.Dsc_inv[e];
    double dres = qv + px;
    dres += aty;
    mx[0] = fmax(mx[0], fabs(dres));      mx[1] = fmax(mx[1], fabs(di * dres));
    mx[2] = fmax(mx[2], fabs(qv));        mx[3] = fmax(mx[3], fabs(aty));   mx[4] = fmax(mx[4], fabs(px));
    mx[5] = fmax(mx[5], fabs(di * qv));   mx[6] = fmax(mx[6], fabs(di * aty)); mx[7] = fmax(mx[7], fabs(di * px));
    sm[0] += 0.5 * xv * px + qv * xv;
  }
  for (int e = tid; e < m * BT; e += nthr) {
    const double ax = p.out1[(size_t)2 * n * BT + e], zv = p.z[e], ei = p.Esc_inv[e];
// ... 2529 lines not shown
  (void)hipGetLastError();
  return best == (1 << 30) ? 0 : best;
}
int max_coresident_factor_groups(int threads, int n_cus) {
  int nb = 0;
  const size_t lds = factor_lds_bytes(1, threads);
  if (hipFuncSetAttribute(reinterpret_cast<const void *>(&factor_kernel<1>), hipFuncAttributeMaxDynamicSharedMemorySize, (int)lds) != hipSuccess ||
      hipOccupancyMaxActiveBlocksPerMultiprocessor(&nb, reinterpret_cast<const void *>(&factor_kernel<1>), threads, lds) != hipSuccess) { (void)hipGetLastError(); return 0; }
  return nb * n_cus;
}

hipError_t launch_advance(const KernelArgs &a, int BT, int tiles, int threads, size_t lds, hipStream_t st, int max_segments, int seg_len,
                          int *host_is, double *host_ds, unsigned *stop, unsigned seq, unsigned *counter, unsigned *host_done) {
  if (a.xs_global || a.wide || a.df || threads > 1024 || (threads > 512 && BT > 2)) return hipErrorInvalidValue;
  AdvanceArgs v{max_segments, seg_len, host_is, host_ds, stop, seq, counter, host_done};
  auto go = [&](auto kern) -> hipError_t {
    hipError_t e = ensure_dynamic_lds(reinterpret_cast<const void *>(kern), lds);
    if (e != hipSuccess) return e;
    hipLaunchKernelGGL(kern, dim3(tiles), dim3(threads), lds, st, a, v);
    return hipGetLastError();
  };
  if (a.rs_off) {
    if (threads <= 512) return hipErrorInvalidValue;
    return BT == 1 ? go(&advance_kernel<1, 1024, true>) : go(&advance_kernel<2, 1024, true>);
  }
  if (threads > 512) return BT == 1 ? go(&advance_kernel<1, 1024>) : go(&advance_kernel<2, 1024>);
  if (BT == 1) return go(&advance_kernel<1, 512>);
  if (BT == 2) return go(&advance_kernel<2, 512>);
  return go(&advance_kernel<4, 512>);
}

static bool grid_form(const KernelArgs &a, int BT, int &tiles, bool from_two, bool need_scratch) {
  if (!a.df || (from_two && a.mw_groups <= 1)) return true;
  if (tiles != 1 || BT != 1 || !a.xs_global || !a.wide || !a.mw_bar || a.mw_groups < 1 || (need_scratch && !a.mw_scratch)) return false;
  tiles = a.mw_groups;
  return true;
}
static bool grid_resident(const void *kern, const KernelArgs &a, int threads, size_t lds, int n_cus) {
  if (!a.df || a.mw_groups <= 1) return true;
  int nb = 0;
  return ensure_dynamic_lds(kern, lds) == hipSuccess && hipOccupancyMaxActiveBlocksPerMultiprocessor(&nb, kern, threads, lds) == hipSuccess &&
         nb * n_cus >= a.mw_groups;
}

int rf_head_steps(int form) { return form == RF_FORM_NONE ? 0 : rf_reg_steps(form) + MI_RF_RL; }
int rf_lds_steps() { return MI_RF_RL; }
hipError_t launch_iterate(const KernelArgs &a, int BT, int tiles, int threads, size_t lds, hipStream_t st) {
  if (getenv("MI_OSQP_DEBUG_HIP")) fprintf(stderr, "[mi_osqp] launch_iterate: df %d wide %d xs_global %p BT %d tiles %d threads %d lds %zu groups %d bar %p\n", a.df, a.wide, (void *)a.xs_global, BT, tiles, threads, lds, a.mw_groups, (void *)a.mw_bar);
  if (!grid_form(a, BT, tiles, false, false)) return hipErrorInvalidValue;
#ifdef MI_OSQP_DEBUG_BUILD
  if (a.df && debug_drop_group("iterate") && tiles > 1) tiles--;
#endif
  if (a.rs_off) {
    if (a.xs_global || a.wide || a.df || threads <= 512 || threads > 1024 || BT > 2) return hipErrorInvalidValue;
    auto go = [&](auto kern) -> hipError_t {
      hipError_t e = ensure_dynamic_lds(reinterpret_cast<const void *>(kern), lds);
      if (e != hipSuccess) return e;
      hipLaunchKernelGGL(kern, dim3(tiles), dim3(threads), lds, st, a);
      return hipGetLastError();
    };
    if (a.rf_off) {
      if (BT != 1 || !a.dt.k || threads != 1024) return hipErrorInvalidValue;
      if (a.rf_form == RF_FORM_LONG_HEAD) return go(&iterate_kernel<1, 1024, false, false, true, RF_FORM_LONG_HEAD>);
      if (a.rf_form == RF_FORM_DEEP_RING) return go(&iterate_kernel<1, 1024, false, false, true, RF_FORM_DEEP_RING>);
      return hipErrorInvalidValue;
    }
    return BT == 1 ? go(&iterate_kernel<1, 1024, false, false, true>) : go(&iterate_kernel<2, 1024, false, false, true>);
  }
  if (a.rf_off) return hipErrorInvalidValue;
  MI_DISPATCH(iterate_kernel, a);
}
hipError_t launch_check(const KernelArgs &a, int BT, int tiles, int threads, size_t lds, hipStream_t st) {
  if (!grid_form(a, BT, tiles, true, true)) return hipErrorInvalidValue;
#ifdef MI_OSQP_DEBUG_BUILD
  if (a.df && a.mw_groups > 1 && debug_drop_group("check") && tiles > 1) tiles--;
#endif
  MI_DISPATCH(check_kernel, a);
}
hipError_t launch_spmv(const KernelArgs &a, int BT, int tiles, int threads, size_t lds, hipStream_t st,
                       const double *x, const double *y, double *Px, double *Aty, double *Ax) {
  MI_DISPATCH(spmv_kernel, a, x, y, Px, Aty, Ax);
}
hipError_t launch_kkt_solve(const KernelArgs &a, int BT, int tiles, int threads, size_t lds, hipStream_t st,
                            const double *rhs, double *sol) {
  if (!grid_form(a, BT, tiles, false, false)) return hipErrorInvalidValue;
#ifdef MI_OSQP_DEBUG_BUILD
  if (a.df && debug_drop_group("kkt") && tiles > 1) tiles--;
#endif
  MI_DISPATCH(kkt_solve_kernel, a, rhs, sol);
}
hipError_t launch_polish_active(const KernelArgs &a, const PolishArgs &p, int BT, hipStream_t st) {
  const size_t total = (size_t)a.B * ((size_t)a.m + 1);
  hipLaunchKernelGGL(polish_active_kernel, dim3((unsigned)((total + 255) / 256)), dim3(256), 0, st, a, p, BT);
  return hipGetLastError();
}
hipError_t launch_polish_active_list(const KernelArgs &a, const PolishArgs &p, const int *slots, int nslots, int BT, hipStream_t st) {
  if (!nslots) return hipSuccess;
  hipLaunchKernelGGL(polish_active_list_kernel, dim3(nslots), dim3(256), 0, st, a, p, slots, BT);
  return hipGetLastError();
}
hipError_t launch_polish_publish(const KernelArgs &a, const PolishArgs &p, const int *slots, int nslots, int *host_stat, int BT, hipStream_t st) {
  if (!nslots) return hipSuccess;
  hipLaunchKernelGGL(polish_publish_kernel, dim3((unsigned)((nslots + 255) / 256)), dim3(256), 0, st, a, p, slots, nslots, host_stat, BT);
  return hipGetLastError();
}
hipError_t launch_polish(const KernelArgs &a, const PolishArgs &p, int BT, int tiles, int threads, size_t lds, int n_cus, hipStream_t st) {
  if (!grid_form(a, BT, tiles, true, true) ||
      !grid_resident(reinterpret_cast<const void *>(&polish_kernel<1, 512, true, true>), a, threads, lds, n_cus)) return hipErrorInvalidValue;
  MI_DISPATCH(polish_kernel, a, p);
}
hipError_t launch_adjoint(const KernelArgs &a, const PolishArgs &p, const AdjointArgs &g, int BT, int tiles, int threads, size_t lds, int n_cus, hipStream_t st) {
  if (!grid_form(a, BT, tiles, true, false) ||
      !grid_resident(reinterpret_cast<const void *>(&adjoint_kernel<1, 512, true, true>), a, threads, lds, n_cus)) return hipErrorInvalidValue;
  MI_DISPATCH(adjoint_kernel, a, p, g);
}
hipError_t launch_adjoint_finish(const int *stat, const AdjointArgs &g, int32_t *status, int B, int n, int m, hipStream_t st) {
  hipLaunchKernelGGL(adjoint_finish_kernel, dim3(B), dim3(256), 0, st, stat, g, status, n, m);
  return hipGetLastError();
}
hipError_t launch_kkt_trace(const KernelArgs &a, int BT, int tiles, int threads, size_t lds, hipStream_t st,
                            const double *rhs, double *sol, uint32_t *trace, uint32_t words) {
  if (BT != 2 || a.xs_global || threads != 512) return hipErrorInvalidValue;
// ... 61 lines not shown
```

### osqp-solver_amd/csrc/sched_format.h

```cpp
#pragma once
#define MI_D_LT(d) ((d) & 7u)
#define MI_D_FLUSH 8u
#define MI_D_TYPE(d) (((d) >> 4) & 3u)
#define MI_D_TYPE_ROW 0u
#define MI_D_NOOP 0x30u
#define MI_D_STORE 0x40u
#define MI_D_PRE 0x80u
#define MI_D_AHEAD 0x100u
#define MI_D_LOOKAHEAD 2
#define MI_D_NBAR(d) ((d) >> 12)
#define MI_D_NBAR_MAX 0xFFFFFu
#define MI_SRC_ZERO (-1)
#define MI_SRC_ONE (-2)
```

### osqp-solver_amd/csrc/solver.hip

```cpp
#include <hip/hip_runtime.h>
#include <time.h>

#include <algorithm>
#include <atomic>
#include <chrono>
#include <cmath>
#include <condition_variable>
#include <functional>
#include <limits>
#include <cstdio>
#include <cstdlib>
#include <cstring>
#include <string>
#include <thread>
#include <map>
#include <memory>
#include <mutex>
#include <vector>

#include "../../include/mi_osqp.h"
#include "device_types.h"
#include "host_core.hpp"

using namespace miosqp;
static_assert((int)kIterStreamed == RF_FORM_NONE && (int)kIterDeepRing == RF_FORM_DEEP_RING && (int)kIterLongHead == RF_FORM_LONG_HEAD, "iterate_form returns RF_FORM_*");

static thread_local std::string g_last_error;

#define HIPCHK(expr)                                                                     \
  do {                                                                                   \
    if (getenv("MI_OSQP_DEBUG_HIP")) {                                                   \
      hipError_t _s = hipGetLastError();                                                 \
      if (_s != hipSuccess) fprintf(stderr, "[mi_osqp] stale HIP error before %s (%s:%d): %s\n", #expr, __FILE__, __LINE__, hipGetErrorString(_s)); \
    }                                                                                    \
    hipError_t _e = (expr);                                                              \
    if (_e != hipSuccess) {                                                              \
      g_last_error = std::string(#expr) + ": " + hipGetErrorString(_e);                  \
      return MI_OSQP_ERR_DEVICE;                                                         \
    }                                                                                    \
  } while (0)

struct DevGuard {
  int prev = -1; bool switched = false;
  explicit DevGuard(int dev) {
    if (hipGetDevice(&prev) == hipSuccess && prev != dev) switched = hipSetDevice(dev) == hipSuccess;
  }
  ~DevGuard() { if (switched) (void)hipSetDevice(prev); }
  DevGuard(const DevGuard &) = delete;
  DevGuard &operator=(const DevGuard &) = delete;
};

static double now_s() {
  return std::chrono::duration<double>(std::chrono::steady_clock::now().time_since_epoch()).count();
}

struct CallTimer {
  struct Slot { const char *name; double s; long calls; };
  static Slot *slots() { static Slot t[16] = {}; return t; }
  static bool on() { static const bool v = getenv("MI_OSQP_DEBUG_TIMING") != nullptr; return v; }
  static void report() {
    for (Slot *t = slots(); t->name; t++) fprintf(stderr, "[mi_osqp] %-28s %6ld calls %9.3f ms\n", t->name, t->calls, 1e3 * t->s);
  }
  const char *name; double t0;
  explicit CallTimer(const char *n) : name(n), t0(on() ? now_s() : 0.0) {}
  ~CallTimer() {
    if (!on()) return;
    static std::mutex mu;
    std::lock_guard<std::mutex> lk(mu);
    Slot *t = slots();
    static bool registered = false;
    if (!registered) { atexit(report); registered = true; }
    while (t->name && t->name != name && t < slots() + 14) t++;
    t->name = name; t->s += now_s() - t0; t->calls++;
  }
};
// ... 133 lines not shown
    if (!count) return 0;
    const size_t bytes = (count * sizeof(T) + 255) & ~(size_t)255;
    if (hipGetDevice(&dev) != hipSuccess) dev = 0;
    if (void *q = devpool::take(dev, bytes, cap)) { p = (T *)q; return 0; }
    hipError_t e = hipMalloc((void **)&p, bytes);
    if (e != hipSuccess) {
      devpool::release_all();
      e = hipMalloc((void **)&p, bytes);
    }
    if (e != hipSuccess) { p = nullptr; g_last_error = std::string("hipMalloc: ") + hipGetErrorString(e); return MI_OSQP_ERR_ALLOC; }
    cap = bytes;
    return 0;
  }
  int zero(hipStream_t s) { if (n && hipMemsetAsync(p, 0, n * sizeof(T), s) != hipSuccess) return MI_OSQP_ERR_DEVICE; return 0; }
  int upload(const std::vector<T> &v) {
    int rc = alloc(v.size());
    if (rc) return rc;
    if (v.size() && hipMemcpy(p, v.data(), v.size() * sizeof(T), hipMemcpyHostToDevice) != hipSuccess) return MI_OSQP_ERR_DEVICE;
    return 0;
  }
  void free() { if (p && !devpool::give(dev, p, cap)) (void)hipFree(p); p = nullptr; n = 0; cap = 0; }
  ~DevBuf() { free(); }
};

struct SchedBufs {
  DevBuf<uint32_t> step, idxw, lvl_pos, tail_bar;
  DevBuf<uint64_t> idxw64;
  DevBuf<int32_t> src;
  int upload(const Schedule &s) {
    int rc;
    if ((rc = step.upload(s.step)) || (rc = idxw.upload(s.idxw)) || (rc = idxw64.upload(s.idxw64)) || (rc = src.upload(s.src)) ||
        (rc = lvl_pos.upload(s.lvl_pos)) || (rc = tail_bar.upload(s.tail_bar))) return rc;
    return 0;
  }
  SchedDev view(const Schedule &s) const {
    SchedDev d; d.step = step.p; d.idxw = idxw.p; d.idxw64 = idxw64.p; d.lvl_pos = lvl_pos.p; d.tail_bar = tail_bar.p;
    d.n_phases = s.n_phases; d.nw = s.nw; d.n_levels = s.n_levels;
    d.n_steps = s.n_steps; d.n_slots = s.n_slots;
    return d;
  }
};

struct mi_osqp_batch {
  Settings st;
  bool rho_interval_auto = false;
  Tuning tune;
  std::shared_ptr<const Analysis> anp;
  int B = 0, BT = 1, ntiles = 0, threads = 512, device = 0, n_cus = 256;
  size_t lds = 0;
  size_t lds_iter = 0;
  int rs_off = 0;
  size_t lds_factor = 0;
  int rf_off = 0, rf_steps = 0;
  int64_t rf_launches[3] = {0, 0, 0};
  std::vector<QPNumeric> qp;
  bool host_bounds_stale = false;
  hipStream_t stream = nullptr;
  SchedBufs fwd, bwd, chk;
  DevBuf<uint32_t> pinv, xloc;
  DevBuf<double> fwd_val, bwd_val, chk_val, dinv, x, z, y, q, l, u, rho_vec, rho_inv, Dsc, Dsc_inv, Esc, Esc_inv;
  DevBuf<double> dx, dy, out1, out2, dscal, x_out, y_out, xs_global;
  DevBuf<double> cert_out;
  bool global_xs = false;
  int mw_groups = 0, mw_threads = 0;
  DevBuf<uint32_t> mw_bar;
  DevBuf<unsigned char> rflag;
  DevBuf<double> mw_scratch;
  DevBuf<double> fwd_val0, bwd_val0, dinv0, rho_vec0, rho_inv0, dscal0;
  DevBuf<int> use_work;
  DevBuf<int> iscal, flag, npos;
  DevBuf<uint32_t> bf_blk, bf_lvl, bf_utask, bf_tri, bf_dtask, bf_ttask, bf_asm_dst, bf_asm_src, bf_ubig;
  DevBuf<int32_t> fwd_srcblk, bwd_srcblk;
  DevBuf<double> pa_val, Lblk, Dl, dinv_scratch;
  DevBuf<uint32_t> dt_task, dt_wave_task, dt_wave_step, dt_tail_bar;
  DevBuf<uint32_t> dt_lt_pos, dt_ltcol_col, dt_tile_tab, dt_wave_tiles, dt_diag_tile, dt_task_step;
  DevBuf<uint64_t> dt_asm_q64;
  DevBuf<int32_t> dt_src_tile;
  int dt_nh = 0; uint32_t dt_cs_doubles = 0; size_t dt_lds = 0, dt_lds_asm = 0;
  DevBuf<int32_t> dt_src;
  DevBuf<double> dt_val, dt_val0, dt_Sd;
  DevBuf<uint32_t> sp_ptr, sp_ent;
  DevBuf<uint32_t> sp_ell, sp_rowid;
  int sp_npass = 0;
  uint32_t sp_ell_off[4] = {0, 0, 0, 0}, sp_ell_k[4] = {0, 0, 0, 0};
  bool host_rho_stale = false;
  bool host_scaling_stale = false;
  DevBuf<int32_t> rz_prow, rz_pcol, rz_arow, rz_acol;
  bool clear_rho_updates = true;
  int *h_npos = nullptr;
  DevBuf<double> stage; DevBuf<int> ids, work;
  int *h_iscal = nullptr;
  double *h_dscal = nullptr;
  size_t h_iscal_cap = 0, h_dscal_cap = 0, h_npos_cap = 0, pin_cap = 0;
  double *pin = nullptr;
  size_t pin_n = 0;
  hipEvent_t ev0 = nullptr, ev1 = nullptr, evf0 = nullptr, evf1 = nullptr, evf2 = nullptr;
  hipStream_t pipe_r = nullptr, pipe_i = nullptr, pipe_x = nullptr;
  hipEvent_t pipe_ev[streampool::kPipeEvents] = {};
  int prio_form = 0, lane_prio = 0, chain_prio = 0;
  bool prio_inert = false;
  hipStream_t pipe_c = nullptr;
  int64_t region_priority = 0, region_lane_checks = 0, region_chunks = 0;
  DevBuf<int> tile_list;
  int64_t pipelined_refactors = 0;
  int64_t refactor_lanes = 0;
  DevBuf<int> ra_list;
// ... 65 lines not shown
    if (pipe_c) (void)hipStreamSynchronize(pipe_c);
    streampool::Bundle sb{device, stream, {ev0, ev1, evf0, evf1, evf2}, pipe_r, pipe_i, pipe_x, {}, lane_prio, pipe_c};
    for (int k = 0; k < streampool::kPipeEvents; k++) sb.pipe_ev[k] = pipe_ev[k];
    if (stream && ev0 && ev1 && evf0 && evf1 && evf2) streampool::give(sb);
    else streampool::destroy(sb);
  }
};

struct mi_osqp_solver { mi_osqp_batch *b = nullptr; };


static Settings to_settings(const mi_osqp_settings *s) {
  Settings t;
  if (!s) return t;
  t.rho = s->rho; t.sigma = s->sigma; t.scaling = s->scaling; t.adaptive_rho = s->adaptive_rho;
  t.adaptive_rho_interval = s->adaptive_rho_interval; t.adaptive_rho_tolerance = s->adaptive_rho_tolerance;
  t.max_iter = s->max_iter; t.eps_abs = s->eps_abs; t.eps_rel = s->eps_rel; t.eps_prim_inf = s->eps_prim_inf;
  t.eps_dual_inf = s->eps_dual_inf; t.alpha = s->alpha; t.scaled_termination = s->scaled_termination;
  t.check_termination = s->check_termination; t.warm_start = s->warm_start; t.verbose = s->verbose;
  t.polish = s->polish; t.polish_refine_iter = s->polish_refine_iter; t.delta = s->delta;
  return t;
}

static void dense_tail_deal_stats(const DenseTail &dt, mi_osqp_stats &s) {
  s.dense_tail_tasks = s.dense_tail_waves_used = s.dense_tail_wave_tasks_max = 0;
  if (!dt.k) return;
  s.dense_tail_tasks = (int64_t)dt.task.size() / 4;
  for (int w = 0; w < dt.nw; w++) {
    const int64_t c = (int64_t)dt.wave_task[w + 1] - (int64_t)dt.wave_task[w];
    s.dense_tail_waves_used += c > 0; s.dense_tail_wave_tasks_max = std::max(s.dense_tail_wave_tasks_max, c);
  }
}

static size_t lds_bytes(int N, int BT, int threads) {
  int nw = threads / 64;
  return ((size_t)N * BT + (size_t)nw * 14 * BT + 14 * BT) * sizeof(double);
}

static KernelArgs make_args(mi_osqp_batch *h) {
  KernelArgs a{};
  a.n = (*h->anp).n; a.m = (*h->anp).m; a.N = (*h->anp).N; a.B = h->B;
  a.fwd = h->fwd.view((*h->anp).fwd); a.bwd = h->bwd.view((*h->anp).bwd); a.chk = h->chk.view((*h->anp).chk);
  a.pinv = h->pinv.p; a.xloc = h->xloc.p;
  a.fwd_val = h->fwd_val.p; a.bwd_val = h->bwd_val.p; a.chk_val = h->chk_val.p; a.dinv = h->dinv.p;
  a.fwd_val0 = h->fwd_val0.p; a.bwd_val0 = h->bwd_val0.p; a.dt_val0 = h->dt_val0.p;
  a.use_work = (h->fwd_val0.p && h->bwd_val0.p && (!(*h->anp).dt.k || h->dt_val0.p)) ? h->use_work.p : nullptr;
  a.x = h->x.p; a.z = h->z.p; a.y = h->y.p; a.q = h->q.p; a.l = h->l.p; a.u = h->u.p;
  a.rho_vec = h->rho_vec.p; a.rho_inv = h->rho_inv.p; a.Dsc = h->Dsc.p; a.Dsc_inv = h->Dsc_inv.p;
  a.Esc = h->Esc.p; a.Esc_inv = h->Esc_inv.p; a.dx = h->dx.p; a.dy = h->dy.p; a.out1 = h->out1.p; a.out2 = h->out2.p;
  a.dscal = h->dscal.p; a.iscal = h->iscal.p;
  a.x_out = h->x_out.p; a.y_out = h->y_out.p;
  a.cert_out = h->cert_out.p; a.cert_stride = (int)std::max<int64_t>(std::max<int64_t>(a.n, a.m), 1);
  a.xs_global = h->global_xs ? h->xs_global.p : nullptr; a.xs_len = (*h->anp).xs_total; a.wide = (*h->anp).wide ? 1 : 0;
  a.rs_off = h->rs_off; a.rf_off = h->rf_off;
  a.rf_form = iterate_form(h->ntiles, h->rf_off != 0, h->tune);
  a.mw_groups = h->mw_groups; a.mw_bar = h->mw_bar.p; a.mw_scratch = h->mw_scratch.p;
  a.df = (*h->anp).df ? 1 : 0; a.df_shadow = (unsigned)(*h->anp).Next; a.rflag = h->rflag.p;
  {
    const DenseTail &dt = (*h->anp).dt;
    a.dt.s = dt.s; a.dt.k = dt.k; a.dt.n_phases = dt.n_phases; a.dt.n_steps = dt.n_steps;
    a.dt.task = h->dt_task.p; a.dt.wave_task = h->dt_wave_task.p; a.dt.wave_step = h->dt_wave_step.p; a.dt.tail_bar = h->dt_tail_bar.p;
    a.dt_val = h->dt_val.p;
  }
  const Settings &s = h->st;
  a.sigma = s.sigma; a.alpha = s.alpha; a.eps_abs = s.eps_abs; a.eps_rel = s.eps_rel;
  a.eps_prim_inf = s.eps_prim_inf; a.eps_dual_inf = s.eps_dual_inf; a.rho_tolerance = s.adaptive_rho_tolerance;
  a.check_termination = (int)s.check_termination; a.rho_interval = (int)s.adaptive_rho_interval;
  a.max_iter = (int)s.max_iter; a.scaled_termination = (int)s.scaled_termination; a.scaling = s.scaling ? 1 : 0;
  a.adaptive_rho = (int)s.adaptive_rho; a.iter_begin = 0; a.iter_end = 0; a.info_at_end = 1;
  return a;
}

static FactorArgs make_factor_args(mi_osqp_batch *h, int force_all) {
  FactorArgs a{};
  const Analysis &an = (*h->anp);
  a.n = an.n; a.m = an.m; a.N = an.N; a.B = h->B; a.nnzP = an.Pp[an.n]; a.nnzK = an.nnzK();
  a.pa_len = an.Pp[an.n] + an.Ap[an.n]; a.n_levels = an.bf.n_levels; a.force_all = force_all;
  a.storage = an.bf.storage; a.fwd = h->fwd.view(an.fwd); a.bwd = h->bwd.view(an.bwd);
  a.blk = h->bf_blk.p; a.lvl = h->bf_lvl.p; a.utask = h->bf_utask.p; a.tri4 = h->bf_tri.p; a.dtask = h->bf_dtask.p; a.ubig = h->bf_ubig.p;
  a.ttask = h->bf_ttask.p; a.asm_dst = h->bf_asm_dst.p; a.asm_src = h->bf_asm_src.p;
  a.fwd_srcblk = h->fwd_srcblk.p; a.bwd_srcblk = h->bwd_srcblk.p;
  a.pa_val = h->pa_val.p; a.l = h->l.p; a.u = h->u.p; a.dscal = h->dscal.p;
  a.rho_vec = h->rho_vec.p; a.rho_inv = h->rho_inv.p; a.Lblk = h->Lblk.p; a.Dl = h->Dl.p; a.dinv_scratch = h->dinv_scratch.p;
  a.fwd_val = h->fwd_val.p; a.bwd_val = h->bwd_val.p; a.dinv = h->dinv.p; a.iscal = h->iscal.p; a.npos = h->npos.p; a.use_work = h->use_work.p;
  a.sigma = h->st.sigma; a.home_bt = h->BT; a.dt_k = an.dt.k;
  a.mw_groups = 0; a.mw_bar = h->mw_bar.p;
#ifdef MI_OSQP_DEBUG_BUILD
  { const char *e = getenv("MI_OSQP_FACTOR_SKIP"); a.debug_skip = e ? atoi(e) : 0; }
#endif
  return a;
}

static int ensure_stage(mi_osqp_batch *h, size_t doubles, size_t ints) {
  int rc;
  if (h->stage.n < doubles && (rc = h->stage.alloc(doubles))) return rc;
  if (h->ids.n < ints && (rc = h->ids.alloc(ints))) return rc;
  return 0;
}

static int ensure_pin(mi_osqp_batch *h, size_t doubles) {
  if (h->pin_n >= doubles) return 0;
  if (h->pin) { hostpool::give(h->pin, h->pin_cap); h->pin = nullptr; h->pin_n = 0; }
  HIPCHK(hostpool::alloc((void **)&h->pin, doubles * sizeof(double), &h->pin_cap));
  h->pin_n = h->pin_cap / sizeof(double);
  return 0;
}
static void par_copy(double *dst, const double *src, size_t n) {
// ... 329 lines not shown
  const Analysis &an = (*h->anp);
  h->B = (int)B;
  h->failed.assign((size_t)B, 0);
  int ndev = 0;
  if (hipGetDeviceCount(&ndev) != hipSuccess || ndev <= 0) { g_last_error = "no HIP device visible"; return MI_OSQP_ERR_DEVICE; }
  if (device >= ndev) { g_last_error = "no such HIP device"; return MI_OSQP_ERR_DEVICE; }
  if (device >= 0) h->device = (int)device; else HIPCHK(hipGetDevice(&h->device));
  DevGuard guard(h->device);
  hipDeviceProp_t prop;
  HIPCHK(hipGetDeviceProperties(&prop, h->device));
  h->n_cus = prop.multiProcessorCount > 0 ? prop.multiProcessorCount : 256;
  if (strncmp(prop.gcnArchName, "gfx950", 6) != 0) { g_last_error = std::string("device is not gfx950: ") + prop.gcnArchName; return MI_OSQP_ERR_DEVICE; }
  {
    streampool::Bundle sb;
    const bool pooled = streampool::take(h->device, sb);
    if (pooled) {
      h->stream = sb.stream; h->ev0 = sb.ev[0]; h->ev1 = sb.ev[1]; h->evf0 = sb.ev[2]; h->evf1 = sb.ev[3]; h->evf2 = sb.ev[4];
      h->pipe_r = sb.pipe_r; h->pipe_i = sb.pipe_i; h->pipe_x = sb.pipe_x; h->pipe_c = sb.pipe_c;
      for (int k = 0; k < streampool::kPipeEvents; k++) h->pipe_ev[k] = sb.pipe_ev[k];
    }
    else {
      HIPCHK(hipStreamCreateWithFlags(&h->stream, hipStreamNonBlocking));
      HIPCHK(hipEventCreate(&h->ev0)); HIPCHK(hipEventCreate(&h->ev1));
      HIPCHK(hipEventCreate(&h->evf0)); HIPCHK(hipEventCreate(&h->evf1)); HIPCHK(hipEventCreate(&h->evf2));
    }
    int least = 0, greatest = 0;
    HIPCHK(hipDeviceGetStreamPriorityRange(&least, &greatest));
    const int asked = h->tune.region_priority;
    h->prio_inert = (asked == 1 && least == 0) || (asked == 2 && greatest == 0);
    h->prio_form = h->prio_inert ? 0 : asked;
    h->lane_prio = h->prio_form == 1 ? least : 0;
    h->chain_prio = greatest;
    if (pooled && sb.lane_prio != h->lane_prio)
      for (hipStream_t *st : {&h->pipe_r, &h->pipe_i, &h->pipe_x}) if (*st) { (void)hipStreamDestroy(*st); *st = nullptr; }
  }
  h->BT = BT; h->ntiles = (int)((B + BT - 1) / BT);
  h->lds = h->global_xs ? lds_bytes(0, BT, h->threads) : lds_bytes(an.Next + 2 * an.dt.k, BT, h->threads);
  if (h->lds > lds_cap) { g_last_error = "internal: LDS budget exceeded"; return MI_OSQP_ERR_ALLOC; }
  h->lds_iter = h->lds; h->rs_off = 0;
  {
    const size_t state = sizeof(double) * (size_t)BT * (2 * (size_t)n + 6 * (size_t)m + (size_t)an.N);
    if (!h->tune.stream_state && !h->global_xs && h->mw_groups <= 0 && h->threads == 1024 && h->lds + state <= lds_cap) {
      h->rs_off = (int)(h->lds / sizeof(double)); h->lds_iter = h->lds + state;
    }
  }
  h->lds_factor = 0; h->rf_off = 0; h->rf_steps = 0;
  if (h->rs_off && BT == 1 && an.dt.k > 0 && !h->tune.stream_factor) {
    const size_t part = (size_t)(h->threads / 64) * rf_lds_steps() * 64 * sizeof(double);
    if (h->lds_iter + part <= lds_cap) {
      h->rf_off = (int)(h->lds_iter / sizeof(double)); h->lds_factor = part;
      h->rf_steps = rf_head_steps(h->tune.rf_form == kIterDeepRing ? RF_FORM_DEEP_RING : RF_FORM_LONG_HEAD);
    }
  }
  size_t T = (size_t)h->ntiles * BT;
  if ((rc = h->fwd.upload(an.fwd)) || (rc = h->bwd.upload(an.bwd)) || (rc = h->chk.upload(an.chk))) return rc;
  { std::vector<uint32_t> pv(an.pinv.begin(), an.pinv.end()); if ((rc = h->pinv.upload(pv))) return rc; }
  { std::vector<uint32_t> xv(an.xloc.begin(), an.xloc.end()); if ((rc = h->xloc.upload(xv))) return rc; }
  {
    std::vector<int32_t> pr(an.Pi.begin(), an.Pi.begin() + an.Pp[n]), pc(an.Pp[n]), ar(an.Ai.begin(), an.Ai.begin() + an.Ap[n]), ac(an.Ap[n]);
    for (int j = 0; j < n; j++) { for (int k = an.Pp[j]; k < an.Pp[j + 1]; k++) pc[k] = j; for (int k = an.Ap[j]; k < an.Ap[j + 1]; k++) ac[k] = j; }
    if ((rc = h->rz_prow.upload(pr)) || (rc = h->rz_pcol.upload(pc)) || (rc = h->rz_arow.upload(ar)) || (rc = h->rz_acol.upload(ac))) return rc;
  }
  if ((rc = h->use_work.alloc(T)) || (rc = h->use_work.zero(h->stream))) return rc;
#define ALLOC(buf, len) if ((rc = h->buf.alloc((size_t)(len) * T)) || (rc = h->buf.zero(h->stream))) return rc
  ALLOC(fwd_val, (size_t)an.fwd.phys_steps() * 64); ALLOC(bwd_val, (size_t)an.bwd.phys_steps() * 64); ALLOC(chk_val, (size_t)an.chk.phys_steps() * 64); ALLOC(dinv, an.N);
  ALLOC(x, n); ALLOC(z, m); ALLOC(y, m); ALLOC(q, n); ALLOC(l, m); ALLOC(u, m); ALLOC(rho_vec, m); ALLOC(rho_inv, m);
  ALLOC(Dsc, n); ALLOC(Dsc_inv, n); ALLOC(Esc, m); ALLOC(Esc_inv, m); ALLOC(dx, n); ALLOC(dy, m);
  ALLOC(out1, 2 * n + m); ALLOC(out2, 2 * n + m); ALLOC(dscal, DS_COUNT);
  if (h->global_xs) { ALLOC(xs_global, an.xs_total); }
  if ((rc = h->mw_bar.alloc(4 * (size_t)std::max(h->n_cus, 1))) || (rc = h->mw_bar.zero(h->stream))) return rc;
  if (an.df && ((rc = h->rflag.upload(an.rflag)) || (rc = h->mw_scratch.alloc((size_t)8 * 256 * 16)) || (rc = h->mw_scratch.zero(h->stream)))) return rc;
  if (an.dt.k) {
    const DenseTail &dt = an.dt;
    ALLOC(dt_val, (size_t)dt.n_steps * 64);
    if ((rc = h->dt_task.upload(dt.task)) || (rc = h->dt_wave_task.upload(dt.wave_task)) || (rc = h->dt_wave_step.upload(dt.wave_step)) ||
        (rc = h->dt_tail_bar.upload(dt.tail_bar)) || (rc = h->dt_src.upload(dt.src)) ||
        (rc = h->dt_lt_pos.upload(dt.lt_pos)) || (rc = h->dt_ltcol_col.upload(dt.ltcol_col)) || (rc = h->dt_tile_tab.upload(dt.tile_tab)) ||
        (rc = h->dt_wave_tiles.upload(dt.wave_tiles)) || (rc = h->dt_asm_q64.upload(dt.asm_q64)) ||
        (rc = h->dt_src_tile.upload(dt.src_tile)) || (rc = h->dt_diag_tile.upload(dt.diag_tile)) || (rc = h->dt_task_step.upload(dt.task_step)) ||
        (rc = h->dt_Sd.alloc((size_t)dt.k * dt.k * (T + 4)))) return rc;
    const int nrt = dt.k / 16 - 4;
    h->dt_nh = nrt <= 14 ? std::max(nrt, 1) : (nrt + 1) / 2;
    h->dt_cs_doubles = (uint32_t)std::max(h->dt_nh * 1024, 64 * 65 + 63) / 64 * 64;
    h->dt_lds = std::max<size_t>((size_t)h->dt_cs_doubles + 4096, 2 * 64 * 65) * sizeof(double);
    h->dt_lds_asm = (dt.asm_lds_bytes() + 255) & ~(size_t)255;
    if (h->dt_lds > lds_cap || h->dt_lds_asm > lds_cap) { g_last_error = "internal: LDS budget of tail_kernel exceeded"; return MI_OSQP_ERR_ALLOC; }
  }
#undef ALLOC
  if ((rc = h->iscal.alloc((size_t)IS_COUNT * T)) || (rc = h->flag.alloc(4))) return rc;
  {
    const BlockFactor &bf = an.bf;
    if ((rc = h->bf_blk.upload(bf.blk)) || (rc = h->bf_lvl.upload(bf.lvl)) || (rc = h->bf_ubig.upload(bf.ubig)) || (rc = h->bf_utask.upload(bf.utask4)) ||
        (rc = h->bf_tri.upload(bf.tri4)) || (rc = h->bf_dtask.upload(bf.dtask4)) || (rc = h->bf_ttask.upload(bf.ttask4)) ||
        (rc = h->bf_asm_dst.upload(bf.asm_dst)) || (rc = h->bf_asm_src.upload(bf.asm_src)) ||
        (rc = h->fwd_srcblk.upload(an.fwd_srcblk)) || (rc = h->bwd_srcblk.upload(an.bwd_srcblk))) return rc;
    if ((rc = h->pa_val.alloc((size_t)(an.Pp[n] + an.Ap[n]) * T)) || (rc = h->pa_val.zero(h->stream)) ||
        (rc = h->Lblk.alloc((size_t)bf.storage * (T + 4))) || (rc = h->Dl.alloc((size_t)an.N * (T + 4))) || (rc = h->Dl.zero(h->stream)) ||
        (rc = h->dinv_scratch.alloc((size_t)an.N * (T + 4))) || (rc = h->npos.alloc(T))) return rc;
    HIPCHK(hostpool::alloc((void **)&h->h_npos, T * sizeof(int), &h->h_npos_cap));
  }
  if (!h->global_xs && an.Pp[n] + an.Ap[n] < 65536 && n + m < 65536 &&
      spmv_fused_lds_bytes((int)n, (int)m, an.Pp[n] + an.Ap[n], BT) <= 150 * 1024) {
    const int nnzP = an.Pp[n];
    std::vector<std::vector<uint32_t>> rows((size_t)2 * n + m);
    for (int c = 0; c < (int)n; c++)
      for (int k = an.Pp[c]; k < an.Pp[c + 1]; k++) {
// ... 94 lines not shown
    size_t cnt = (size_t)DS_COUNT * T;
    for (size_t k = 0; k < cnt; k++) h->h_dscal[k] = 0.0;
    HIPCHK(hipMemcpy(h->dscal.p, h->h_dscal, cnt * sizeof(double), hipMemcpyHostToDevice));
    if ((rc = sync_scalars_to_device(h, all, !dev_ruiz))) return rc;
  }
  if (dev_ruiz) {
    double tb = now_s();
    const size_t cA = (size_t)B * nnzA, cb = (size_t)B * m, cpa = (size_t)B * (an.Pp[n] + nnzA);
    if ((rc = ensure_pin(h, cA + 2 * cb + 1)) || (rc = ensure_stage(h, cA + 2 * cb + cpa + 1, (size_t)B))) return rc;
    par_copy(h->pin, Av, cA);
    if (m) { par_copy(h->pin + cA, l, cb); par_copy(h->pin + cA + cb, u, cb); }
    HIPCHK(hipMemcpyAsync(h->stage.p, h->pin, (cA + 2 * cb) * sizeof(double), hipMemcpyHostToDevice, h->stream));
    RuizArgs r{};
    r.n = (int)n; r.m = (int)m; r.nnzP = an.Pp[n]; r.nnzA = nnzA; r.B = (int)B; r.BT = BT; r.iters = (int)h->st.scaling;
    r.ids = nullptr; r.fresh = 1; r.rawP = h->rawP.p; r.rawq = h->rawq.p;
    r.Prow = h->rz_prow.p; r.Pcol = h->rz_pcol.p; r.Arow = h->rz_arow.p; r.Acol = h->rz_acol.p;
    r.rawA = h->stage.p; r.rawl = h->stage.p + cA; r.rawu = h->stage.p + cA + cb;
    r.pa_val = h->pa_val.p; r.q = h->q.p; r.Dsc = h->Dsc.p; r.Dsc_inv = h->Dsc_inv.p; r.Esc = h->Esc.p; r.Esc_inv = h->Esc_inv.p;
    r.l = h->l.p; r.u = h->u.p; r.dscal = h->dscal.p;
    r.dn = h->out1.p; r.en = h->out1.p + (size_t)B * n;
    r.pa_out = h->stage.p + cA + 2 * cb;
    HIPCHK(launch_ruiz(r, h->stream));
    std::vector<int> ids(B);
    for (int i = 0; i < (int)B; i++) ids[i] = i;
    HIPCHK(hipMemcpyAsync(h->ids.p, ids.data(), ids.size() * sizeof(int), hipMemcpyHostToDevice, h->stream));
    HIPCHK(launch_scatter(r.pa_out, h->chk_val.p, h->chk.src.p, h->ids.p, (int)B, an.Pp[n] + nnzA, h->chk.view(an.chk), BT, h->stream));
    HIPCHK(hipStreamSynchronize(h->stream));
    h->host_scaling_stale = true; h->host_bounds_stale = true; h->host_rho_stale = true;
    t_factor += now_s() - tb;
  }
  {
    double tb = now_s();
    std::vector<int> all(B);
    for (int i = 0; i < (int)B; i++) all[i] = i;
    if ((rc = refactor_qps(h, std::move(all)))) return rc;
    t_factor += now_s() - tb;
  }
  if ((rc = reset_solve_state(h, true))) return rc;
  if ((rc = snapshot(h))) return rc;
  HIPCHK(hipStreamSynchronize(h->stream));
  mi_osqp_stats &s = h->stats;
  s.n = n; s.m = m; s.N = an.N; s.batch = B; s.tile = BT; s.n_tiles = h->ntiles;
  s.nnz_P_triu = an.Pp[n]; s.nnz_A = nnzA; s.nnz_KKT = an.nnzK(); s.nnz_L = an.nnzL();
  s.n_supernodes = (int64_t)an.sn_start.size() - 1; s.n_blocks = (int64_t)an.chunk_start.size() - 1;
  s.fwd_levels = an.fwd.n_phases; s.bwd_levels = an.bwd.n_phases;
  s.fwd_slots = (int64_t)an.fwd.phys_steps() * 64; s.bwd_slots = (int64_t)an.bwd.phys_steps() * 64; s.chk_slots = (int64_t)an.chk.phys_steps() * 64;
  s.lds_bytes = (int64_t)h->lds; s.threads_per_block = h->threads;
  s.dense_tail_rows = an.dt.k; s.dense_tail_slots = (int64_t)an.dt.n_steps * 64;
  s.setup_seconds_host = t1 - t0; s.setup_seconds_factor = t_factor; s.setup_seconds_upload = t_upload;
  s.nnz_L_before_tail = an.dt.k ? an.Lp[an.dt.s] : an.nnzL();
  s.solve_groups = h->mw_groups; s.solve_group_threads = h->mw_groups > 0 ? h->mw_threads : 0;
  s.resident_state = h->rs_off ? 1 : 0; s.lds_bytes_iterate = (int64_t)h->lds_iter;
  s.resident_factor_steps = h->rf_steps; s.lds_bytes_factor = (int64_t)h->lds_factor;
  dense_tail_deal_stats(an.dt, s);
  if (getenv("MI_OSQP_DEBUG_TIMING"))
    fprintf(stderr, "[mi_osqp] setup B=%d N=%d: analysis+alloc %.1f ms (analysis %.1f), numeric %.1f ms, upload %.1f ms, rest %.1f ms\n", (int)B, an.N,
            1e3 * (t1 - t0), 1e3 * t_analysis, 1e3 * t_factor, 1e3 * t_upload, 1e3 * (now_s() - t1 - t_factor - t_upload));
  return MI_OSQP_OK;
}


static int fail_slots(mi_osqp_batch *h, const KernelArgs &a, const std::vector<int> &bad, int iter) {
  if (bad.empty()) return 0;
  int rc;
  if (h->fail_list.n < bad.size() && (rc = h->fail_list.alloc(std::max<size_t>(bad.size(), (size_t)h->ntiles * h->BT)))) return rc;
  HIPCHK(hipMemcpyAsync(h->fail_list.p, bad.data(), bad.size() * sizeof(int), hipMemcpyHostToDevice, h->stream));
  HIPCHK(launch_fail_slots(a, h->fail_list.p, (int)bad.size(), h->BT, iter, h->stream));
  HIPCHK(hipStreamSynchronize(h->stream));
  for (int q : bad) if (q >= 0 && q < h->B) h->failed[q] = 1;
  return 0;
}

static TailArgs make_tail_args(mi_osqp_batch *h, int kbt, const int *work) {
  const DenseTail &dt = (*h->anp).dt;
  TailArgs da{};
  da.n = (*h->anp).n; da.N = (*h->anp).N; da.s = dt.s; da.k = dt.k; da.kbt = kbt; da.home_bt = h->BT;
  da.storage = (*h->anp).bf.storage; da.n_slots = dt.n_steps * 64u; da.n_lt = dt.n_lt; da.n_ltcol = dt.n_ltcol; da.n_quads = (uint32_t)(dt.asm_q64.size() / 64);
  da.nh = h->dt_nh; da.cs_doubles = h->dt_cs_doubles; da.work = work;
  da.lt_pos = h->dt_lt_pos.p; da.ltcol_col = h->dt_ltcol_col.p; da.tile_tab = h->dt_tile_tab.p; da.wave_tiles = h->dt_wave_tiles.p;
  da.dt_task = h->dt_task.p; da.dt_task_step = h->dt_task_step.p; da.n_tasks = (uint32_t)(dt.task.size() / 4);
  da.asm_q64 = h->dt_asm_q64.p; da.diag_tile = h->dt_diag_tile.p; da.src_tile = h->dt_src_tile.p;
  da.Lblk = h->Lblk.p; da.Dl = h->Dl.p; da.Sd = h->dt_Sd.p; da.dt_val = h->dt_val.p; da.dinv = h->dinv.p; da.npos = h->npos.p; da.iscal = h->iscal.p;
  return da;
}

static void to_polish_factor(mi_osqp_batch *h, const PolishArgs &pol, FactorArgs &fa, TailArgs &da) {
  fa.pmask = pol.act; fa.arow = h->rz_arow.p; fa.pstat = pol.stat; fa.pdelta = h->st.delta; fa.sigma = h->st.delta;
  fa.fwd_val = h->pol_fwd.p; fa.bwd_val = h->pol_bwd.p; fa.dinv = h->pol_dinv.p; fa.use_work = nullptr;
  da.dt_val = h->pol_dt.p; da.dinv = h->pol_dinv.p; da.pstat = pol.stat;
}
static KernelArgs polish_stream_args(mi_osqp_batch *h, KernelArgs a) {
  a.fwd_val = h->pol_fwd.p; a.bwd_val = h->pol_bwd.p; a.dinv = h->pol_dinv.p; a.dt_val = h->pol_dt.p; a.use_work = nullptr;
  return a;
}
static std::vector<int> koptimal_slots(const mi_osqp_batch *h) {
  const int BT = h->BT;
  std::vector<int> work;
  for (int q = 0; q < h->B; q++)
    if (h->h_iscal[(size_t)(q / BT) * IS_COUNT * BT + IS_STATUS * BT + q % BT] == 1) work.push_back(q);
  return work;
}

static int device_refactor_slots(mi_osqp_batch *h, std::vector<int> work, std::vector<int> *bad, const PolishArgs *pol = nullptr) {
  if (work.empty()) return 0;
  const int BT = h->BT;
  int rc;
// ... 2582 lines not shown
int mi_osqp_debug_refactor_lanes(int64_t n_flagged, const int64_t *flagged, int64_t n_active, const int64_t *active, int64_t tile,
                                 int64_t chunk_qps, int64_t max_chunks, int64_t kbt, int64_t lanes, int64_t chunk0_first,
                                 int64_t scratch_slots, int64_t *n_lanes, int64_t *lane_of, int64_t *order, int64_t *order_begin,
                                 int64_t *scratch_begin, int64_t *n_waits, int64_t *wait_chunk, int64_t *wait_for) {
  if (!n_lanes || !lane_of || !order || !order_begin || !scratch_begin || !n_waits || !wait_chunk || !wait_for ||
      (n_flagged > 0 && !flagged) || (n_active > 0 && !active)) return MI_OSQP_ERR_NULL;
  if (n_flagged < 0 || n_active < 0 || tile < 1 || chunk_qps < 1 || max_chunks < 1 || kbt < 1 || lanes < 1 || lanes > 3 || scratch_slots < 0)
    return MI_OSQP_ERR_INVALID_DATA;
  const std::vector<int> f(flagged, flagged + n_flagged), a(active, active + n_active);
  const RefactorChunks ch = refactor_chunks(f, a, (int)tile, (int)chunk_qps, (int)max_chunks);
  const RefactorLanes rl = refactor_lanes(ch, f, (int)tile, (int)kbt, (int)lanes, chunk0_first != 0, (int)std::min<int64_t>(scratch_slots, INT32_MAX));
  *n_lanes = rl.n_lanes;
  std::copy(rl.lane_of.begin(), rl.lane_of.end(), lane_of);
  order_begin[0] = 0;
  for (int l = 0; l < rl.n_lanes; l++) {
    std::copy(rl.order[l].begin(), rl.order[l].end(), order + order_begin[l]);
    order_begin[l + 1] = order_begin[l] + (int64_t)rl.order[l].size();
  }
  std::copy(rl.scratch_begin.begin(), rl.scratch_begin.begin() + ch.n_chunks, scratch_begin);
  *n_waits = (int64_t)rl.wait_chunk.size();
  std::copy(rl.wait_chunk.begin(), rl.wait_chunk.end(), wait_chunk);
  std::copy(rl.wait_for.begin(), rl.wait_for.end(), wait_for);
  return MI_OSQP_OK;
}
int mi_osqp_debug_runahead_group(int64_t n_active, const int64_t *tiles, const double *pri_res, const double *dua_res, int64_t size,
                                 int64_t min_active, int64_t *n_group, int64_t *group) {
  if (!n_group || !group || (n_active > 0 && (!tiles || !pri_res || !dua_res))) return MI_OSQP_ERR_NULL;
  if (n_active < 0 || n_active > INT32_MAX || size < 0 || size > INT32_MAX || min_active < 0 || min_active > INT32_MAX) return MI_OSQP_ERR_INVALID_DATA;
  std::vector<int> t((size_t)n_active);
  for (int64_t i = 0; i < n_active; i++) {
    if (tiles[i] < 0 || tiles[i] > INT32_MAX || pri_res[i] < 0.0 || dua_res[i] < 0.0) return MI_OSQP_ERR_INVALID_DATA;
    t[(size_t)i] = (int)tiles[i];
  }
  {
    std::vector<int> sorted = t;
    std::sort(sorted.begin(), sorted.end());
    if (std::adjacent_find(sorted.begin(), sorted.end()) != sorted.end()) return MI_OSQP_ERR_INVALID_DATA;
  }
  const std::vector<int> g = runahead_group(t, std::vector<double>(pri_res, pri_res + n_active), std::vector<double>(dua_res, dua_res + n_active),
                                            (int)size, (int)min_active);
  *n_group = (int64_t)g.size();
  std::copy(g.begin(), g.end(), group);
  return MI_OSQP_OK;
}
int mi_osqp_debug_iterate_form(int64_t tiles, int64_t has_head, int64_t forced_form, int64_t long_min, int64_t *form) {
  if (!form) return MI_OSQP_ERR_NULL;
  if (tiles < 0 || tiles > INT32_MAX || forced_form < 0 || forced_form > 2 || long_min < -1 || long_min > INT32_MAX)
    return MI_OSQP_ERR_INVALID_DATA;
  Tuning t;
  t.rf_form = (int)forced_form; t.rf_long_min = (int)long_min;
  *form = iterate_form((int)tiles, has_head != 0, t);
  return MI_OSQP_OK;
}
int mi_osqp_get_stats(mi_osqp_solver *h, mi_osqp_stats *st) { return h ? mi_osqp_batch_get_stats(h->b, st) : MI_OSQP_ERR_NULL; }
int mi_osqp_get_settings(mi_osqp_solver *h, mi_osqp_settings *out) { return h ? mi_osqp_batch_get_settings(h->b, out) : MI_OSQP_ERR_NULL; }
int mi_osqp_update_settings(mi_osqp_solver *h, const mi_osqp_settings *s) { return h ? mi_osqp_batch_update_settings(h->b, s) : MI_OSQP_ERR_NULL; }


}

struct ShardWorker {
  std::thread th;
  std::mutex mu;
  std::condition_variable cv;
  std::function<int()> job;
  bool has_job = false, busy = false, quit = false;
  int rc = 0;
  std::string err;
  void start() {
    th = std::thread([this] {
      std::unique_lock<std::mutex> lk(mu);
      for (;;) {
        cv.wait(lk, [this] { return has_job || quit; });
        if (quit) return;
        std::function<int()> f = std::move(job);
        has_job = false;
        lk.unlock();
        const int r = f();
        const std::string e = r ? g_last_error : std::string();
        lk.lock();
        rc = r; err = e; busy = false;
        cv.notify_all();
      }
    });
  }
  void post(std::function<int()> f) {
    std::unique_lock<std::mutex> lk(mu);
    cv.wait(lk, [this] { return !busy; });
    job = std::move(f); has_job = true; busy = true; rc = 0; err.clear();
    cv.notify_all();
  }
  int wait(std::string &e) {
    std::unique_lock<std::mutex> lk(mu);
    cv.wait(lk, [this] { return !busy; });
    e = err;
    return rc;
  }
  ~ShardWorker() {
    { std::lock_guard<std::mutex> lk(mu); quit = true; }
    cv.notify_all();
    if (th.joinable()) th.join();
  }
};

struct mi_osqp_multi {
  int64_t B = 0, n = 0, m = 0;
// ... 258 lines not shown
```

Baseline: 46000.

## Keep per-thread xloc/pinv index words in registers across ADMM iterations

```diff
diff --git a/include/mi_osqp.h b/include/mi_osqp.h
--- a/include/mi_osqp.h
+++ b/include/mi_osqp.h
@@ -85,6 +85,8 @@
   int64_t iterate_launches_deep_ring, iterate_launches_long_head;
   int64_t runahead_regions, runahead_tiles, runahead_left, runahead_missed;
   int64_t region_priority, region_lane_checks, region_chunks;
+  int64_t ring_early;
+  int64_t resident_index_words;
 } mi_osqp_stats;
 
 typedef struct mi_osqp_solver mi_osqp_solver;
@@ -308,6 +310,9 @@
 
 int mi_osqp_debug_iterate_form(int64_t tiles, int64_t has_head, int64_t forced_form, int64_t long_min, int64_t *form);
 
+int mi_osqp_debug_index_words_fit(int64_t resident_state, int64_t lds_vector, int64_t tile, int64_t threads, int64_t n, int64_t m,
+                                  int64_t *fit, int64_t *xloc_trips, int64_t *pinv_trips);
+
 int mi_osqp_debug_trace_kkt_solve(mi_osqp_batch *h, int32_t which, const double *d_rhs, double *d_sol,
                                   uint32_t *out, int64_t out_capacity_words, int64_t *dims);
 
diff --git a/osqp-solver_amd/__init__.py b/osqp-solver_amd/__init__.py
--- a/osqp-solver_amd/__init__.py
+++ b/osqp-solver_amd/__init__.py
@@ -53,7 +53,8 @@
                 ("iterate_launches_deep_ring", C.c_int64), ("iterate_launches_long_head", C.c_int64),
                 ("runahead_regions", C.c_int64), ("runahead_tiles", C.c_int64), ("runahead_left", C.c_int64),
                 ("runahead_missed", C.c_int64),
-                ("region_priority", C.c_int64), ("region_lane_checks", C.c_int64), ("region_chunks", C.c_int64)]
+                ("region_priority", C.c_int64), ("region_lane_checks", C.c_int64), ("region_chunks", C.c_int64),
+                ("ring_early", C.c_int64), ("resident_index_words", C.c_int64)]
 
     def as_dict(self):
         return {k: getattr(self, k) for k, _ in self._fields_}
@@ -196,6 +197,7 @@
         L.mi_osqp_debug_runahead_group.argtypes = [C.c_int64, ip, dp, dp, C.c_int64, C.c_int64, ip, ip]
         L.mi_osqp_debug_region_chunks.argtypes = [C.c_int64] * 3 + [ip] * 2
         L.mi_osqp_debug_iterate_form.argtypes = [C.c_int64] * 4 + [ip]
+        L.mi_osqp_debug_index_words_fit.argtypes = [C.c_int64] * 6 + [ip] * 3
         L.mi_osqp_prefetch_analysis.argtypes = [C.c_int64, C.c_int64, C.c_int64, ip, ip, ip, ip, C.c_int64]
         L.mi_osqp_debug_host_block_factor.argtypes = [C.c_int64, C.c_int64, ip, ip, dp, ip, ip, dp, dp, dp,
                                                       C.POINTER(Settings), dp, dp, ip]
@@ -881,6 +883,13 @@
     return int(form.value)
 
 
+def debug_index_words_fit(n, m, tile=1, threads=1024, resident_state=True, lds_vector=True):
+    fit, xt, pt = C.c_int64(), C.c_int64(), C.c_int64()
+    _chk(lib().mi_osqp_debug_index_words_fit(int(bool(resident_state)), int(bool(lds_vector)), tile, threads, n, m,
+                                             C.byref(fit), C.byref(xt), C.byref(pt)), "debug_index_words_fit")
+    return bool(fit.value), int(xt.value), int(pt.value)
+
+
 def debug_host_block_factor(P, A, l, u, **settings):
     L = lib()
     P, A = _csc(P), _csc(A)
diff --git a/osqp-solver_amd/csrc/device_types.h b/osqp-solver_amd/csrc/device_types.h
--- a/osqp-solver_amd/csrc/device_types.h
+++ b/osqp-solver_amd/csrc/device_types.h
@@ -48,6 +48,8 @@
   int rs_off;
   int rf_off;
   int rf_form;
+  int ix;
+  int re;
   int wide;
   double sigma, alpha, eps_abs, eps_rel, eps_prim_inf, eps_dual_inf, rho_tolerance;
   int check_termination, rho_interval, max_iter, scaled_termination, scaling, adaptive_rho;
diff --git a/osqp-solver_amd/csrc/host_core.cpp b/osqp-solver_amd/csrc/host_core.cpp
--- a/osqp-solver_amd/csrc/host_core.cpp
+++ b/osqp-solver_amd/csrc/host_core.cpp
@@ -958,6 +958,8 @@
   if (const char *e = getenv("MI_OSQP_RUNAHEAD_END")) t.runahead_end = std::max(0, atoi(e));
   if (const char *e = getenv("MI_OSQP_RF_FORM")) { const int v = atoi(e); if (v == kIterDeepRing || v == kIterLongHead) t.rf_form = v; }
   if (const char *e = getenv("MI_OSQP_RF_LONG_MIN")) t.rf_long_min = std::max(0, atoi(e));
+  if (const char *e = getenv("MI_OSQP_INDEX_LOADS")) t.index_loads = atoi(e) != 0;
+  if (const char *e = getenv("MI_OSQP_RING_EARLY")) t.ring_early = atoi(e) != 0;
   AnalysisTuning &a = t.analysis;
   if (const char *e = getenv("MI_OSQP_DENSE_TAIL")) a.dense_tail = atoi(e);
   if (const char *e = getenv("MI_OSQP_ORDERING")) a.ordering = e[0];
@@ -1070,6 +1072,12 @@
   if (t.rf_form == kIterDeepRing || t.rf_form == kIterLongHead) return t.rf_form;
   const int long_min = t.rf_long_min >= 0 ? t.rf_long_min : kRfLongMinDefault;
   return tiles > 0 && tiles >= long_min ? kIterLongHead : kIterDeepRing;
+}
+
+bool index_words_fit(bool resident_state, bool lds_vector, int bt, int threads, int64_t n, int64_t m) {
+  if (!resident_state || !lds_vector || bt < 1 || threads < 64 || n < 1 || m < 0) return false;
+  const int64_t xcap = (int64_t)MI_IX_XLOC_TRIPS * threads, pcap = (int64_t)MI_IX_PINV_TRIPS * threads;
+  return (n + m) * bt <= xcap && n * bt <= pcap && m * bt <= pcap;
 }
 
 
diff --git a/osqp-solver_amd/csrc/host_core.hpp b/osqp-solver_amd/csrc/host_core.hpp
--- a/osqp-solver_amd/csrc/host_core.hpp
+++ b/osqp-solver_amd/csrc/host_core.hpp
@@ -38,6 +38,7 @@
 constexpr bool kRunaheadDefault = true;
 constexpr int kRegionPriorityDefault = 0;
 constexpr bool kLaneChecksDefault = false;
+constexpr bool kRingEarlyDefault = false;
 struct Tuning {
   int tile = 0;
   int threads = 0;
@@ -66,9 +67,13 @@
   int runahead_end = 0;
   int rf_form = 0;
   int rf_long_min = -1;
+  bool index_loads = false;
+  bool ring_early = kRingEarlyDefault;
   AnalysisTuning analysis;
 };
 Tuning tuning_from_env();
+
+bool index_words_fit(bool resident_state, bool lds_vector, int bt, int threads, int64_t n, int64_t m);
 
 enum IterateForm { kIterStreamed = 0, kIterDeepRing = 1, kIterLongHead = 2 };
 constexpr int kRfLongMinDefault = 0;
diff --git a/osqp-solver_amd/csrc/kernels.hip b/osqp-solver_amd/csrc/kernels.hip
--- a/osqp-solver_amd/csrc/kernels.hip
+++ b/osqp-solver_amd/csrc/kernels.hip
@@ -203,18 +203,32 @@
   return pos + (uint32_t)lane < end ? d : MI_D_NOOP;
 }
 
-template <int BT, int PF, bool SUB, bool BAR, bool GX, int TR = 0, bool WIDE = false>
+template <int BT, int PF, bool WIDE>
+__device__ __forceinline__ void ring_start(const ValSrc<BT> &vs, uint32_t begin, uint32_t end, int lane, Ring<BT, PF> &r) {
+  r.desc = load_desc(vs, begin, end, lane);
+#pragma unroll
+  for (int st = 0; st < PF; st++) {
+    r.gr[st] = 0u;
+    load_step<BT, WIDE>(vs, begin + (uint32_t)st, lane, r.v[st], r.gi[st], r.gr[st]);
+  }
+}
+
+template <int BT, int PF, bool SUB, bool BAR, bool GX, int TR = 0, bool WIDE = false, bool PRE = false>
 __device__ __forceinline__ void run_stream(const ValSrc<BT> &vs, uint32_t begin, uint32_t end, uint32_t tail, double *xs,
                                            double *out, int lane, uint32_t *tr = nullptr, int wave = 0, int nw = 0,
-                                           uint32_t *tw = nullptr) {
+                                           uint32_t *tw = nullptr, const Ring<BT, PF> *pre = nullptr) {
   double *base = SUB ? xs : out;
   Ring<BT, PF> r;
-  r.desc = MI_D_NOOP;
-#pragma unroll
-  for (int st = 0; st < PF; st++) {
-    r.gi[st] = 0u; r.gr[st] = 0u;
-#pragma unroll
-    for (int b = 0; b < BT; b++) r.v[st][b] = 0.0;
+  if constexpr (PRE) {
+    r = *pre;
+  } else {
+    r.desc = MI_D_NOOP;
+#pragma unroll
+    for (int st = 0; st < PF; st++) {
+      r.gi[st] = 0u; r.gr[st] = 0u;
+#pragma unroll
+      for (int b = 0; b < BT; b++) r.v[st][b] = 0.0;
+    }
   }
   constexpr uint32_t NONE = WIDE ? 0xFFFFFFFFu : 0xFFFFu;
   static_assert(PF % (MI_D_LOOKAHEAD + 1) == 0, "the gather slots must line up across ring revolutions");
@@ -232,7 +246,7 @@
     if constexpr (GX) __syncthreads(); else lds_barrier();
     if constexpr (TR) { if (lane == 0) tr[((size_t)nbar_seen * nw + wave) * 2 + 1] = (uint32_t)__builtin_amdgcn_s_memtime(); nbar_seen++; }
   };
-  for (uint32_t npos = begin; npos < end + PF; npos += PF) {
+  for (uint32_t npos = PRE ? begin + PF : begin; npos < end + PF; npos += PF) {
     const uint32_t dnext = load_desc(vs, npos, end, lane);
 #pragma unroll
     for (int st = 0; st < PF; st++) {
@@ -447,6 +461,17 @@
   if constexpr (GX && TR == 0 && BT <= 2) run_stream_gx<BT, MI_GX_PF, MI_GX_LA, WIDE>(vals, begin, end, tail, xs, lane);
   else run_stream<BT, PF, true, true, GX, TR, WIDE>(vals, begin, end, tail, xs, nullptr, lane, tr, wave, s.nw, tw);
 }
+template <int BT, int PF>
+__device__ __forceinline__ void tri_start(const SchedDev &s, const ValSrc<BT> &vals, int wave, int lane, Ring<BT, PF> &r) {
+  mi_cptr lp = as_const(s.lvl_pos);
+  ring_start<BT, PF, false>(vals, lp[wave], lp[(size_t)s.n_levels * s.nw + wave], lane, r);
+}
+template <int BT, int PF>
+__device__ __forceinline__ void tri_finish(const SchedDev &s, const ValSrc<BT> &vals, double *xs, int wave, int lane, const Ring<BT, PF> &r) {
+  mi_cptr lp = as_const(s.lvl_pos);
+  const uint32_t begin = lp[wave], end = lp[(size_t)s.n_levels * s.nw + wave], tail = as_const(s.tail_bar)[wave];
+  run_stream<BT, PF, true, true, false, 0, false, true>(vals, begin, end, tail, xs, nullptr, lane, nullptr, wave, s.nw, nullptr, &r);
+}
 
 template <int BT, int PF, bool WIDE = false>
 __device__ __forceinline__ void run_spmv(const SchedDev &s, const ValSrc<BT> &vals, double *xs, double *out, int wave,
@@ -657,9 +682,10 @@
 #endif
 __host__ __device__ constexpr int rf_reg_steps(int RF) { return RF == RF_FORM_LONG_HEAD ? MI_RF_R_LONG : RF == RF_FORM_DEEP_RING ? MI_RF_R_DEEP : 1; }
 __host__ __device__ constexpr int rf_ring_steps(int RF) { return RF == RF_FORM_LONG_HEAD ? MI_RF_PF_LONG : MI_RF_PF_DEEP; }
-template <int R, int RL, int PF>
+struct NoEarly { __device__ __forceinline__ void operator()() const {} };
+template <int R, int RL, int PF, class F = NoEarly>
 __device__ __forceinline__ void dense_tail_apply_rf(const DenseTailDev &dt, const mi_rsrc &vals, const double *xt, double *yr, double *yc,
-                                                    double (&keep)[R], double *hl, bool first, int wave, int lane) {
+                                                    double (&keep)[R], double *hl, bool first, int wave, int lane, F early = F{}) {
   constexpr int H = R + RL;
   static_assert(H % PF == 0 && H <= 32 && RL <= PF, "the head is whole ring revolutions inside the shortest task");
   mi_cptr tk = as_const(dt.task);
@@ -734,34 +760,63 @@
       if (left == 0) flush();
     }
   }
+  early();
   for (uint32_t nb = as_const(dt.tail_bar)[wave]; nb; nb--) lds_barrier();
 }
 
-template <int BT, bool GX>
+struct IxWords { uint32_t x[(MI_IX_XLOC_TRIPS + 1) / 2], p[MI_IX_PINV_TRIPS]; };
+__device__ __forceinline__ uint32_t ix_pos(uint32_t w, bool high) { return high ? w >> 16 : (w & 0xFFFFu); }
+__device__ __forceinline__ int ix_opaque(int tid) { asm volatile("" : "+v"(tid)); return tid; }
+
+template <int BT, bool GX, bool IX = false, bool RE = false, class F = NoEarly>
 __device__ __forceinline__ void kkt_middle(const KernelArgs &a, const double *dinv, const mi_rsrc (&vdt)[BT], int act, double *xs,
-                                           int tid, int nthr, int wave, int lane) {
+                                           int tid, int nthr, int wave, int lane, const IxWords &ix = IxWords{}, F early = F{}) {
+  static_assert(!IX || !GX, "the index words are LDS positions");
+  static_assert(!RE || IX, "an index load behind the early ring would wait for all of it");
   if (!a.dt.k) {
-    constexpr int U = GX ? 8 : 1;
     const int tot = a.N * BT;
-    for (int e0 = tid; e0 < tot; e0 += nthr * U) {
-      size_t pos[U]; double v[U], dv[U];
-#pragma unroll
-      for (int u = 0; u < U; u++) { const int e = e0 + u * nthr < tot ? e0 + u * nthr : e0; pos[u] = (size_t)a.xloc[e / BT] * BT + e % BT; dv[u] = dinv[e]; }
-#pragma unroll
-      for (int u = 0; u < U; u++) v[u] = xs[pos[u]];
-#pragma unroll
-      for (int u = 0; u < U; u++) if (e0 + u * nthr < tot) xs[pos[u]] = v[u] * dv[u];
-    }
-    __syncthreads();
+    if constexpr (IX) {
+      if constexpr (RE) early();
+      const int t0 = ix_opaque(tid);
+#pragma unroll
+      for (int j = 0; j < MI_IX_XLOC_TRIPS; j++) {
+        const int e = t0 + j * nthr;
+        if (e < tot) { const uint32_t pos = ix_pos(ix.x[j / 2], j & 1); const double v = xs[pos]; xs[pos] = v * dinv[e]; }
+      }
+    } else {
+      constexpr int U = GX ? 8 : 1;
+      for (int e0 = tid; e0 < tot; e0 += nthr * U) {
+        size_t pos[U]; double v[U], dv[U];
+#pragma unroll
+        for (int u = 0; u < U; u++) { const int e = e0 + u * nthr < tot ? e0 + u * nthr : e0; pos[u] = (size_t)a.xloc[e / BT] * BT + e % BT; dv[u] = dinv[e]; }
+#pragma unroll
+        for (int u = 0; u < U; u++) v[u] = xs[pos[u]];
+#pragma unroll
+        for (int u = 0; u < U; u++) if (e0 + u * nthr < tot) xs[pos[u]] = v[u] * dv[u];
+      }
+    }
+    if constexpr (RE) lds_barrier(); else __syncthreads();
     return;
   }
   if constexpr (!GX) {
     const int s = a.dt.s, k = a.dt.k;
     double *yr = xs + (size_t)a.xs_len * BT, *yc = yr + (size_t)k * BT;
-    for (int e = tid; e < a.N * BT; e += nthr) {
-      const int i = e / BT;
-      if (i < s) xs[(size_t)a.xloc[i] * BT + e % BT] *= dinv[e];
-      else { yr[e - s * BT] = dinv[e] * xs[e]; yc[e - s * BT] = 0.0; }
+    if constexpr (IX) {
+      const int t0 = ix_opaque(tid);
+#pragma unroll
+      for (int j = 0; j < MI_IX_XLOC_TRIPS; j++) {
+        const int e = t0 + j * nthr;
+        if (e < a.N * BT) {
+          if (e / BT < s) xs[ix_pos(ix.x[j / 2], j & 1)] *= dinv[e];
+          else { yr[e - s * BT] = dinv[e] * xs[e]; yc[e - s * BT] = 0.0; }
+        }
+      }
+    } else {
+      for (int e = tid; e < a.N * BT; e += nthr) {
+        const int i = e / BT;
+        if (i < s) xs[(size_t)a.xloc[i] * BT + e % BT] *= dinv[e];
+        else { yr[e - s * BT] = dinv[e] * xs[e]; yc[e - s * BT] = 0.0; }
+      }
     }
     __syncthreads();
     if constexpr (BT == 1) {
@@ -775,26 +830,41 @@
         dense_tail_apply<BT, BT, MI_DT_PF>(a.dt, vdt, 0, xs + (size_t)s * BT, yr, yc, wave, lane);
       }
     }
+    if constexpr (RE) early();
     for (int e = tid; e < k * BT; e += nthr) xs[(size_t)s * BT + e] = yr[e] + yc[e];
-    __syncthreads();
-  }
-}
-
-template <int R, int RL, int PF>
+    if constexpr (RE) lds_barrier(); else __syncthreads();
+  }
+}
+
+template <int R, int RL, int PF, bool IX = false, bool RE = false, class F = NoEarly>
 __device__ __forceinline__ void kkt_middle_rf(const KernelArgs &a, const double *dinv, const mi_rsrc &vdt, double *xs, double (&keep)[R],
-                                              double *hl, bool first, int tid, int nthr, int wave, int lane) {
+                                              double *hl, bool first, int tid, int nthr, int wave, int lane, const IxWords &ix = IxWords{},
+                                              F early = F{}) {
+  static_assert(!RE || IX, "an index load behind the early ring would wait for all of it");
   const int s = a.dt.s, k = a.dt.k;
   double *yr = xs + (size_t)a.xs_len, *yc = yr + (size_t)k;
-  int e0 = tid;
-  asm volatile("" : "+v"(e0));
-  for (int e = e0; e < a.N; e += nthr) {
-    if (e < s) xs[(size_t)a.xloc[e]] *= dinv[e];
-    else { yr[e - s] = dinv[e] * xs[e]; yc[e - s] = 0.0; }
+  if constexpr (IX) {
+    const int t0 = ix_opaque(tid);
+#pragma unroll
+    for (int j = 0; j < MI_IX_XLOC_TRIPS; j++) {
+      const int e = t0 + j * nthr;
+      if (e < a.N) {
+        if (e < s) xs[ix_pos(ix.x[j / 2], j & 1)] *= dinv[e];
+        else { yr[e - s] = dinv[e] * xs[e]; yc[e - s] = 0.0; }
+      }
+    }
+  } else {
+    int e0 = tid;
+    asm volatile("" : "+v"(e0));
+    for (int e = e0; e < a.N; e += nthr) {
+      if (e < s) xs[(size_t)a.xloc[e]] *= dinv[e];
+      else { yr[e - s] = dinv[e] * xs[e]; yc[e - s] = 0.0; }
+    }
   }
   __syncthreads();
-  dense_tail_apply_rf<R, RL, PF>(a.dt, vdt, xs + (size_t)s, yr, yc, keep, hl, first, wave, lane);
+  dense_tail_apply_rf<R, RL, PF>(a.dt, vdt, xs + (size_t)s, yr, yc, keep, hl, first, wave, lane, early);
   for (int e = tid; e < k; e += nthr) xs[(size_t)s + e] = yr[e] + yc[e];
-  __syncthreads();
+  if constexpr (RE) lds_barrier(); else __syncthreads();
 }
 
 __device__ __forceinline__ uint32_t df_floc(uint32_t e, uint32_t f, uint32_t xl, uint32_t sh) { return (f & 4u) ? xl : ((f & 1u) ? e + sh : e); }
@@ -841,9 +911,11 @@
   run_tri<BT, PF, GX, 0, WIDE>(a.bwd, p.vbwd, xs, wave, lane);
 }
 
-template <int BT, int NT, bool GX, bool WIDE = false, bool RS = false, int RF = 0>
+template <int BT, int NT, bool GX, bool WIDE = false, bool RS = false, int RF = 0, bool IX = false, bool RE = false>
 __device__ __forceinline__ void iterate_body(const KernelArgs &a, double *smem, int n_iter) {
   static_assert(!RS || (!GX && !WIDE), "the resident state goes with the LDS solve vector");
+  static_assert(!IX || RS, "the index words in registers go with the resident state");
+  static_assert(!RE || (IX && BT == 1), "the early rings go with the index words in registers of a tile of one QP");
   static_assert(!RF || (RS && BT == 1 && NT == 1024), "the resident head goes with the resident state of a 16-wave tile of one QP");
   const Mw mw{a.mw_bar, GX && BT == 1 && a.mw_groups > 1 ? (unsigned)a.mw_groups : 1u};
   const bool multi = GX && BT == 1 && mw.G > 1;
@@ -873,6 +945,27 @@
   double *hl = nullptr;
   (void)keep; (void)hl;
   if constexpr (RF) hl = smem + a.rf_off + (size_t)(wave * MI_RF_RL) * 64 + lane;
+  IxWords ix{};
+  (void)ix;
+  if constexpr (IX) {
+#pragma unroll
+    for (int j = 0; j < MI_IX_XLOC_TRIPS; j++) {
+      const int e = tid + j * nthr;
+      const uint32_t w = e < N * BT ? a.xloc[e / BT] * (uint32_t)BT + (uint32_t)b : 0u;
+      ix.x[j / 2] |= w << (16 * (j & 1));
+    }
+#pragma unroll
+    for (int j = 0; j < MI_IX_PINV_TRIPS; j++) {
+      const int e = tid + j * nthr;
+      const uint32_t wx = e < n * BT ? a.pinv[e / BT] * (uint32_t)BT + (uint32_t)b : 0u;
+      const uint32_t wz = e < m * BT ? a.pinv[n + e / BT] * (uint32_t)BT + (uint32_t)b : 0u;
+      ix.p[j] = wx | (wz << 16);
+    }
+  }
+  constexpr int PFS = MI_PFV_NT(NT, GX);
+  Ring<BT, PFS> rfw, rbw;
+  (void)rfw; (void)rbw;
+  if constexpr (RE) tri_start<BT, PFS>(a.fwd, p.vfwd, wave, lane, rfw);
   for (int e = tid; e < N * BT; e += nthr) {
     const int i = e / BT;
     double v;
@@ -900,19 +993,64 @@
   for (int iter = 1; iter <= n_iter; iter++) {
     const bool do_info = a.info_at_end && iter == n_iter;
     const bool last = iter == n_iter;
-    if constexpr (RS) {
+    if constexpr (RE) {
+      auto early = [&]() { tri_start<BT, PFS>(a.bwd, p.vbwd, wave, lane, rbw); };
+      tri_finish<BT, PFS>(a.fwd, p.vfwd, xs, wave, lane, rfw);
+      if constexpr (RF) kkt_middle_rf<rf_reg_steps(RF), MI_RF_RL, rf_ring_steps(RF), true, true>(a, DI, p.vdt[0], xs, keep, hl, iter == 1, tid, nthr, wave, lane, ix, early);
+      else kkt_middle<BT, false, true, true>(a, DI, p.vdt, p.act, xs, tid, nthr, wave, lane, ix, early);
+      tri_finish<BT, PFS>(a.bwd, p.vbwd, xs, wave, lane, rbw);
+      if (!last) tri_start<BT, PFS>(a.fwd, p.vfwd, wave, lane, rfw);
+    } else if constexpr (RS) {
       run_tri<BT, MI_PFV_NT(NT, GX), GX, 0, WIDE>(a.fwd, p.vfwd, xs, wave, lane);
-      if constexpr (RF) kkt_middle_rf<rf_reg_steps(RF), MI_RF_RL, rf_ring_steps(RF)>(a, DI, p.vdt[0], xs, keep, hl, iter == 1, tid, nthr, wave, lane);
-      else kkt_middle<BT, GX>(a, DI, p.vdt, p.act, xs, tid, nthr, wave, lane);
+      if constexpr (RF) kkt_middle_rf<rf_reg_steps(RF), MI_RF_RL, rf_ring_steps(RF), IX>(a, DI, p.vdt[0], xs, keep, hl, iter == 1, tid, nthr, wave, lane, ix);
+      else kkt_middle<BT, GX, IX>(a, DI, p.vdt, p.act, xs, tid, nthr, wave, lane, ix);
       run_tri<BT, MI_PFV_NT(NT, GX), GX, 0, WIDE>(a.bwd, p.vbwd, xs, wave, lane);
     } else {
       kkt_solve_lds<BT, MI_PFV_NT(NT, GX), GX, WIDE>(a, p, xs, tid, nthr, wave, nw, lane, mw);
     }
+    if constexpr (IX) {
+      const int t0 = ix_opaque(tid);
+#pragma unroll
+      for (int j = 0; j < MI_IX_PINV_TRIPS; j++) {
+        const int e = t0 + j * nthr;
+        if (e < n * BT) {
+          const uint32_t pos = ix_pos(ix.p[j], false);
+          const double xt = xs[pos], xp = X[e], qv = Q[e];
+          double xn = alpha * xt + (1.0 - alpha) * xp;
+          if (!done) {
+            X[e] = xn;
+            if (last) p.x[e] = xn;
+            if (do_info) p.dx[e] = xn - xp;
+          } else xn = xp;
+          xs[pos] = sigma * xn - qv;
+        }
+      }
+#pragma unroll
+      for (int j = 0; j < MI_IX_PINV_TRIPS; j++) {
+        const int e = t0 + j * nthr;
+        if (e < m * BT) {
+          const uint32_t pos = ix_pos(ix.p[j], true);
+          const double nu = xs[pos], zp = Z[e], yv = Y[e], ri = RI[e], rv = RV[e], lo = LO[e], up = UP[e];
+          double zt = zp - ri * yv;
+          zt += ri * nu;
+          const double zr = alpha * zt + (1.0 - alpha) * zp;
+          double zn = fmin(fmax(zr + ri * yv, lo), up);
+          const double dyv = rv * (zr - zn);
+          double yn = yv + dyv;
+          if (!done) {
+            Z[e] = zn; Y[e] = yn;
+            if (last) { p.z[e] = zn; p.y[e] = yn; }
+            if (do_info) p.dy[e] = dyv;
+          } else { zn = zp; yn = yv; }
+          xs[pos] = zn - ri * yn;
+        }
+      }
+    }
     constexpr int U = GX ? 4 : 1;
     int tid_i = tid;
-    if constexpr (RF != 0) asm volatile("" : "+v"(tid_i));
+    if constexpr (RF != 0 && !IX) asm volatile("" : "+v"(tid_i));
     uint32_t fl[U], xl[U];
-    for (int e0 = tid_i; e0 < n * BT; e0 += nthr * U) {
+    if constexpr (!IX) for (int e0 = tid_i; e0 < n * BT; e0 += nthr * U) {
       size_t pos[U]; double xt[U], xp[U], qv[U];
 #pragma unroll
       for (int u = 0; u < U; u++) { const int e = e0 + u * nthr < n * BT ? e0 + u * nthr : e0; pos[u] = (size_t)a.pinv[e / BT] * BT + b; }
@@ -940,7 +1078,7 @@
         }
       }
     }
-    for (int e0 = tid_i; e0 < m * BT; e0 += nthr * U) {
+    if constexpr (!IX) for (int e0 = tid_i; e0 < m * BT; e0 += nthr * U) {
       size_t pos[U]; double nu[U], zp[U], yv[U], ri[U], rv[U], lo[U], up[U];
 #pragma unroll
       for (int u = 0; u < U; u++) { const int e = e0 + u * nthr < m * BT ? e0 + u * nthr : e0; pos[u] = (size_t)a.pinv[n + e / BT] * BT + b; }
@@ -973,13 +1111,15 @@
         }
       }
     }
-    if constexpr (GX) wg_or_grid_barrier(mw); else __syncthreads();
-  }
-}
-template <int BT, int NT, bool GX, bool WIDE = false, bool RS = false, int RF = 0>
+    if constexpr (GX) wg_or_grid_barrier(mw);
+    else if constexpr (RE) lds_barrier();
+    else __syncthreads();
+  }
+}
+template <int BT, int NT, bool GX, bool WIDE = false, bool RS = false, int RF = 0, bool IX = false, bool RE = false>
 __global__ __launch_bounds__(NT) void iterate_kernel(KernelArgs a) {
   extern __shared__ double smem[];
-  iterate_body<BT, NT, GX, WIDE, RS, RF>(a, smem, a.iter_end - a.iter_begin);
+  iterate_body<BT, NT, GX, WIDE, RS, RF, IX, RE>(a, smem, a.iter_end - a.iter_begin);
 }
 
 template <int BT, int NT, bool GX, bool WIDE = false>
@@ -3615,7 +3755,7 @@
   if (a.df && debug_drop_group("iterate") && tiles > 1) tiles--;
 #endif
   if (a.rs_off) {
-    if (a.xs_global || a.wide || a.df || threads <= 512 || threads > 1024 || BT > 2) return hipErrorInvalidValue;
+    if (a.xs_global || a.wide || a.df || threads <= 512 || threads > 1024 || BT > 2 || (a.re && (!a.ix || BT != 1))) return hipErrorInvalidValue;
     auto go = [&](auto kern) -> hipError_t {
       hipError_t e = ensure_dynamic_lds(reinterpret_cast<const void *>(kern), lds);
       if (e != hipSuccess) return e;
@@ -3624,13 +3764,18 @@
     };
     if (a.rf_off) {
       if (BT != 1 || !a.dt.k || threads != 1024) return hipErrorInvalidValue;
-      if (a.rf_form == RF_FORM_LONG_HEAD) return go(&iterate_kernel<1, 1024, false, false, true, RF_FORM_LONG_HEAD>);
-      if (a.rf_form == RF_FORM_DEEP_RING) return go(&iterate_kernel<1, 1024, false, false, true, RF_FORM_DEEP_RING>);
+      if (a.re && a.rf_form == RF_FORM_DEEP_RING) return go(&iterate_kernel<1, 1024, false, false, true, RF_FORM_DEEP_RING, true, true>);
+      if (a.rf_form == RF_FORM_LONG_HEAD)
+        return a.ix ? go(&iterate_kernel<1, 1024, false, false, true, RF_FORM_LONG_HEAD, true>) : go(&iterate_kernel<1, 1024, false, false, true, RF_FORM_LONG_HEAD>);
+      if (a.rf_form == RF_FORM_DEEP_RING)
+        return a.ix ? go(&iterate_kernel<1, 1024, false, false, true, RF_FORM_DEEP_RING, true>) : go(&iterate_kernel<1, 1024, false, false, true, RF_FORM_DEEP_RING>);
       return hipErrorInvalidValue;
     }
+    if (a.re) return go(&iterate_kernel<1, 1024, false, false, true, 0, true, true>);
+    if (a.ix) return BT == 1 ? go(&iterate_kernel<1, 1024, false, false, true, 0, true>) : go(&iterate_kernel<2, 1024, false, false, true, 0, true>);
     return BT == 1 ? go(&iterate_kernel<1, 1024, false, false, true>) : go(&iterate_kernel<2, 1024, false, false, true>);
   }
-  if (a.rf_off) return hipErrorInvalidValue;
+  if (a.rf_off || a.ix || a.re) return hipErrorInvalidValue;
   MI_DISPATCH(iterate_kernel, a);
 }
 hipError_t launch_check(const KernelArgs &a, int BT, int tiles, int threads, size_t lds, hipStream_t st) {
diff --git a/osqp-solver_amd/csrc/sched_format.h b/osqp-solver_amd/csrc/sched_format.h
--- a/osqp-solver_amd/csrc/sched_format.h
+++ b/osqp-solver_amd/csrc/sched_format.h
@@ -12,3 +12,5 @@
 #define MI_D_NBAR_MAX 0xFFFFFu
 #define MI_SRC_ZERO (-1)
 #define MI_SRC_ONE (-2)
+#define MI_IX_XLOC_TRIPS 2
+#define MI_IX_PINV_TRIPS 1
diff --git a/osqp-solver_amd/csrc/solver.hip b/osqp-solver_amd/csrc/solver.hip
--- a/osqp-solver_amd/csrc/solver.hip
+++ b/osqp-solver_amd/csrc/solver.hip
@@ -21,6 +21,7 @@
 #include "../../include/mi_osqp.h"
 #include "device_types.h"
 #include "host_core.hpp"
+#include "sched_format.h"
 
 using namespace miosqp;
 static_assert((int)kIterStreamed == RF_FORM_NONE && (int)kIterDeepRing == RF_FORM_DEEP_RING && (int)kIterLongHead == RF_FORM_LONG_HEAD, "iterate_form returns RF_FORM_*");
@@ -260,6 +261,8 @@
   int rs_off = 0;
   size_t lds_factor = 0;
   int rf_off = 0, rf_steps = 0;
+  int re = 0;
+  int ix = 0;
   int64_t rf_launches[3] = {0, 0, 0};
   std::vector<QPNumeric> qp;
   bool host_bounds_stale = false;
@@ -431,7 +434,7 @@
   a.x_out = h->x_out.p; a.y_out = h->y_out.p;
   a.cert_out = h->cert_out.p; a.cert_stride = (int)std::max<int64_t>(std::max<int64_t>(a.n, a.m), 1);
   a.xs_global = h->global_xs ? h->xs_global.p : nullptr; a.xs_len = (*h->anp).xs_total; a.wide = (*h->anp).wide ? 1 : 0;
-  a.rs_off = h->rs_off; a.rf_off = h->rf_off;
+  a.rs_off = h->rs_off; a.rf_off = h->rf_off; a.ix = h->ix; a.re = h->re;
   a.rf_form = iterate_form(h->ntiles, h->rf_off != 0, h->tune);
   a.mw_groups = h->mw_groups; a.mw_bar = h->mw_bar.p; a.mw_scratch = h->mw_scratch.p;
   a.df = (*h->anp).df ? 1 : 0; a.df_shadow = (unsigned)(*h->anp).Next; a.rflag = h->rflag.p;
@@ -867,6 +870,8 @@
       h->rf_steps = rf_head_steps(h->tune.rf_form == kIterDeepRing ? RF_FORM_DEEP_RING : RF_FORM_LONG_HEAD);
     }
   }
+  h->ix = !h->tune.index_loads && index_words_fit(h->rs_off != 0, !h->global_xs, BT, h->threads, n, m) ? 1 : 0;
+  h->re = h->ix && BT == 1 && h->tune.ring_early && (!h->rf_off || h->tune.rf_form == kIterDeepRing) ? 1 : 0;
   size_t T = (size_t)h->ntiles * BT;
   if ((rc = h->fwd.upload(an.fwd)) || (rc = h->bwd.upload(an.bwd)) || (rc = h->chk.upload(an.chk))) return rc;
   { std::vector<uint32_t> pv(an.pinv.begin(), an.pinv.end()); if ((rc = h->pinv.upload(pv))) return rc; }
@@ -1067,6 +1072,7 @@
   s.solve_groups = h->mw_groups; s.solve_group_threads = h->mw_groups > 0 ? h->mw_threads : 0;
   s.resident_state = h->rs_off ? 1 : 0; s.lds_bytes_iterate = (int64_t)h->lds_iter;
   s.resident_factor_steps = h->rf_steps; s.lds_bytes_factor = (int64_t)h->lds_factor;
+  s.ring_early = h->re; s.resident_index_words = h->ix;
   dense_tail_deal_stats(an.dt, s);
   if (getenv("MI_OSQP_DEBUG_TIMING"))
     fprintf(stderr, "[mi_osqp] setup B=%d N=%d: analysis+alloc %.1f ms (analysis %.1f), numeric %.1f ms, upload %.1f ms, rest %.1f ms\n", (int)B, an.N,
@@ -3755,6 +3761,15 @@
   *form = iterate_form((int)tiles, has_head != 0, t);
   return MI_OSQP_OK;
 }
+int mi_osqp_debug_index_words_fit(int64_t resident_state, int64_t lds_vector, int64_t tile, int64_t threads, int64_t n, int64_t m,
+                                  int64_t *fit, int64_t *xloc_trips, int64_t *pinv_trips) {
+  if (!fit || !xloc_trips || !pinv_trips) return MI_OSQP_ERR_NULL;
+  if ((tile != 1 && tile != 2 && tile != 4) || threads < 64 || threads > 1024 || threads % 64 || n < 1 || m < 0 || n + m > (int64_t)1 << 30)
+    return MI_OSQP_ERR_INVALID_DATA;
+  *fit = index_words_fit(resident_state != 0, lds_vector != 0, (int)tile, (int)threads, n, m) ? 1 : 0;
+  *xloc_trips = MI_IX_XLOC_TRIPS; *pinv_trips = MI_IX_PINV_TRIPS;
+  return MI_OSQP_OK;
+}
 int mi_osqp_get_stats(mi_osqp_solver *h, mi_osqp_stats *st) { return h ? mi_osqp_batch_get_stats(h->b, st) : MI_OSQP_ERR_NULL; }
 int mi_osqp_get_settings(mi_osqp_solver *h, mi_osqp_settings *out) { return h ? mi_osqp_batch_get_settings(h->b, out) : MI_OSQP_ERR_NULL; }
 int mi_osqp_update_settings(mi_osqp_solver *h, const mi_osqp_settings *s) { return h ? mi_osqp_batch_update_settings(h->b, s) : MI_OSQP_ERR_NULL; }
```

After: 46670, median of 6. 1.5% higher.
